# evandieren/AbstractBayesOpt.jl

Hardware: NVIDIA B200
Metric: candidate posterior+EI evals/sec at n=8192,d=20 (higher is better)
Workload: dtype f64

## Files before the change

abstractbayesopt.jl_b200/csrc/abo_api.cu:

```cuda
#include <algorithm>
#include <cmath>
#include <cstdarg>
#include <cstdio>
#include <cstring>
#include <cstdlib>
#include <limits>
#include <new>
#include <string>
#include <vector>

#include <cuda_runtime.h>

#include "../../include/abo.h"
#include "gemm_dmma.cuh"
#include "kernels.cuh"
#include "sweep_fused.cuh"
#include "gemm_tma.cuh"
#include "sample.cuh"
#include "abo_internal.h"

using namespace abo;

static thread_local std::string g_err;

int abo_fail(int code, const char* fmt, ...) {
    char buf[512];
    va_list ap;
    va_start(ap, fmt);
    vsnprintf(buf, sizeof buf, fmt, ap);
    va_end(ap);
    g_err = buf;
    return code;
}

extern "C" const char* abo_last_error(void) { return g_err.c_str(); }
extern "C" int32_t abo_version(void) { return 100; }

static int configure_kernels() {
    CU(cudaFuncSetAttribute(gemm_dmma_kernel, cudaFuncAttributeMaxDynamicSharedMemorySize, GEMM_SMEM_BYTES));
    CU(cudaFuncSetAttribute(gemm_small_kernel<32, 8>, cudaFuncAttributeMaxDynamicSharedMemorySize, GemmS<32, 8>::SMEM_BYTES));
    CU(cudaFuncSetAttribute(gemm_small_kernel<64, 8>, cudaFuncAttributeMaxDynamicSharedMemorySize, GemmS<64, 8>::SMEM_BYTES));
    CU(cudaFuncSetAttribute(gemm_k128_kernel<16, 128>, cudaFuncAttributeMaxDynamicSharedMemorySize, GemmK128<16, 128>::SMEM_BYTES));
    CU(cudaFuncSetAttribute(gemm_k128_kernel<32, 32>, cudaFuncAttributeMaxDynamicSharedMemorySize, GemmK128<32, 32>::SMEM_BYTES));
    CU(cudaFuncSetAttribute(fill_distance_kernel, cudaFuncAttributeMaxDynamicSharedMemorySize, 256 * 96 * 8));
    CU(cudaFuncSetAttribute(potf2_ws_kernel, cudaFuncAttributeMaxDynamicSharedMemorySize, PW_SMEM_BYTES));
    CU(cudaFuncSetAttribute(syrk_tma_kernel, cudaFuncAttributeMaxDynamicSharedMemorySize, SY_SMEM_BYTES));
    CU(cudaFuncSetAttribute(gemm_tma_kernel<EPI_STORE>, cudaFuncAttributeMaxDynamicSharedMemorySize, tg_smem_bytes<EPI_STORE>()));
    CU(cudaFuncSetAttribute(gemm_tma_kernel<EPI_COLSUMSQ>, cudaFuncAttributeMaxDynamicSharedMemorySize, tg_smem_bytes<EPI_COLSUMSQ>()));
#define ABO_FS_CFG(DT) CU(cudaFuncSetAttribute(sweep_fused_kernel<DT>, cudaFuncAttributeMaxDynamicSharedMemorySize, fused_smem_bytes<DT>()))
    ABO_FS_CFG(4); ABO_FS_CFG(8); ABO_FS_CFG(12); ABO_FS_CFG(16); ABO_FS_CFG(20); ABO_FS_CFG(24); ABO_FS_CFG(32);
#undef ABO_FS_CFG
    return ABO_OK;
}

static int ctx_init_resources(abo_ctx* c) {
    int prio_lo = 0, prio_hi = 0;
    CU(cudaDeviceGetStreamPriorityRange(&prio_lo, &prio_hi));
    CU(cudaStreamCreateWithPriority(&c->stream, cudaStreamNonBlocking, prio_hi));
    CU(cudaStreamCreateWithPriority(&c->stream2, cudaStreamNonBlocking, prio_lo));
    CU(cudaStreamCreateWithPriority(&c->stream3, cudaStreamNonBlocking, prio_hi));
    CU(cudaStreamCreateWithPriority(&c->stream4, cudaStreamNonBlocking, prio_lo));
    CU(cudaEventCreateWithFlags(&c->ev_inv, cudaEventDisableTiming));
    for (int q = 0; q < 3; ++q) CU(cudaEventCreateWithFlags(&c->ev_p[q], cudaEventDisableTiming));
    CU(cudaEventCreateWithFlags(&c->ev_a, cudaEventDisableTiming));
    CU(cudaEventCreateWithFlags(&c->ev_b, cudaEventDisableTiming));
    for (int q = 0; q < 2; ++q) {
        CU(cudaEventCreateWithFlags(&c->ev_h2d[q], cudaEventDisableTiming));
        CU(cudaEventCreateWithFlags(&c->ev_pc[q], cudaEventDisableTiming));
    }
    return configure_kernels();
}

extern "C" int32_t abo_ctx_create(int32_t device, abo_ctx** out) {
    if (!out) return abo_fail(ABO_ERR_INVALID, "abo_ctx_create: out is NULL");
    int ndev = 0;
    cudaError_t e = cudaGetDeviceCount(&ndev);
    if (e != cudaSuccess || ndev == 0)
        return abo_fail(ABO_ERR_CUDA, "no CUDA device available (%s); libabo_cuda has no CPU fallback",
                        e == cudaSuccess ? "device count 0" : cudaGetErrorString(e));
    if (device < 0 || device >= ndev) return abo_fail(ABO_ERR_INVALID, "device %d out of range [0,%d)", device, ndev);
    CU(cudaSetDevice(device));
    cudaDeviceProp prop;
    CU(cudaGetDeviceProperties(&prop, device));
    if (prop.major < 10)
        return abo_fail(ABO_ERR_CUDA, "device %d is sm_%d%d; libabo_cuda is built for sm_100a only", device, prop.major,
                        prop.minor);
    abo_ctx* c = new (std::nothrow) abo_ctx();
    if (!c) return abo_fail(ABO_ERR_ALLOC, "host allocation failed");
    c->device = device;
    c->sms = prop.multiProcessorCount;
    int rc = ctx_init_resources(c);
    if (rc) { abo_ctx_destroy(c); return rc; }
    *out = c;
    return ABO_OK;
}

static void gp_free_device(abo_gp* g);
void ctx_sync_all(abo_ctx* c) {
    for (cudaStream_t s_ : {c->stream, c->stream2, c->stream3, c->stream4}) if (s_) cudaStreamSynchronize(s_);
}

extern "C" int32_t abo_ctx_destroy(abo_ctx* c) {
    if (!c) return ABO_OK;
    const std::string keep = g_err;
    cudaSetDevice(c->device);
    ctx_sync_all(c);
    for (abo_gp* g : c->live) { gp_free_device(g); g->ctx = nullptr; }
    c->live.clear();
    for (auto& b : c->ws) if (b.ptr) cudaFree(b.ptr);
    gp_pool_clear(c);
    for (auto e : c->prof_events) cudaEventDestroy(e);
    if (c->pinned) cudaFreeHost(c->pinned);
    abo_nccl_teardown(c);
    auto ev_free = [](cudaEvent_t e) { if (e) cudaEventDestroy(e); };
    ev_free(c->ev_a); ev_free(c->ev_b);
    for (int q = 0; q < 2; ++q) { ev_free(c->ev_h2d[q]); ev_free(c->ev_pc[q]); }
    for (cudaStream_t s_ : {c->stream, c->stream2, c->stream3, c->stream4}) if (s_) cudaStreamDestroy(s_);
    ev_free(c->ev_inv);
    for (int q = 0; q < 3; ++q) ev_free(c->ev_p[q]);
    cudaGetLastError();
    delete c;
    g_err = keep;
    return ABO_OK;
}

extern "C" int32_t abo_ctx_trim(abo_ctx* c) {
    if (!c) return abo_fail(ABO_ERR_INVALID, "null ctx");
    CU(cudaSetDevice(c->device));
    ctx_sync_all(c);
    gp_pool_clear(c);
    for (auto& b : c->ws) if (b.ptr) { cudaFree(b.ptr); b.ptr = nullptr; b.bytes = 0; }
    if (c->pinned) { cudaFreeHost(c->pinned); c->pinned = nullptr; c->pinned_bytes = 0; }
    return ABO_OK;
}

extern "C" int32_t abo_ctx_device(const abo_ctx* c, int32_t* device) {
    if (!c || !device) return abo_fail(ABO_ERR_INVALID, "null argument");
    *device = c->device;
    return ABO_OK;
}
extern "C" int32_t abo_ctx_stream(const abo_ctx* c, void** stream) {
    if (!c || !stream) return abo_fail(ABO_ERR_INVALID, "null argument");
    *stream = (void*)c->stream;
    return ABO_OK;
}
extern "C" int32_t abo_ctx_launch_count(const abo_ctx* c, int64_t* count) {
    if (!c || !count) return abo_fail(ABO_ERR_INVALID, "null argument");
    *count = c->launches;
    return ABO_OK;
}

int prof_mark(abo_ctx* c) {
    if (!c->profile) return ABO_OK;
    if (c->prof_used == c->prof_events.size()) {
        cudaEvent_t e;
        CU(cudaEventCreate(&e));
        c->prof_events.push_back(e);
    }
    CU(cudaEventRecord(c->prof_events[c->prof_used++], c->stream));
    return ABO_OK;
}
int prof_collect(abo_ctx* c) {
    if (!c->profile) return ABO_OK;
    for (size_t i = 0; i + 1 < c->prof_used; i += 2) {
        float ms = 0;
        CU(cudaEventElapsedTime(&ms, c->prof_events[i], c->prof_events[i + 1]));
        int cls = (int)((i / 2) % 3);
        c->prof_ms[cls] += ms;
        c->prof_n[cls] += 1;
    }
    c->prof_used = 0;
    return ABO_OK;
}
extern "C" int32_t abo_ctx_profile(abo_ctx* c, int32_t enable) {
    if (!c) return abo_fail(ABO_ERR_INVALID, "null ctx");
    CU(cudaSetDevice(c->device));
    CU(cudaStreamSynchronize(c->stream));
    c->profile = enable != 0;
    c->prof_used = 0;
    for (int i = 0; i < 3; ++i) { c->prof_ms[i] = 0; c->prof_n[i] = 0; }
    return ABO_OK;
}
extern "C" int32_t abo_ctx_profile_read(abo_ctx* c, double ms[3], int64_t launches[3]) {
    if (!c || !ms || !launches) return abo_fail(ABO_ERR_INVALID, "null argument");
    CU(cudaSetDevice(c->device));
    CU(cudaStreamSynchronize(c->stream));
    int rc = prof_collect(c);
    if (rc) return rc;
    for (int i = 0; i < 3; ++i) { ms[i] = c->prof_ms[i]; launches[i] = c->prof_n[i]; }
    return ABO_OK;
}

typedef CUresult (*EncodeTiledFn)(CUtensorMap*, CUtensorMapDataType, cuuint32_t, void*, const cuuint64_t*,
                                  const cuuint64_t*, const cuuint32_t*, const cuuint32_t*, CUtensorMapInterleave,
                                  CUtensorMapSwizzle, CUtensorMapL2promotion, CUtensorMapFloatOOBfill);
static EncodeTiledFn get_encode_fn() {
    static EncodeTiledFn fn = nullptr;
    if (!fn) {
        void* ptr = nullptr;
        cudaDriverEntryPointQueryResult q;
        if (cudaGetDriverEntryPoint("cuTensorMapEncodeTiled", &ptr, cudaEnableDefault, &q) == cudaSuccess &&
            q == cudaDriverEntryPointSuccess)
            fn = (EncodeTiledFn)ptr;
    }
    return fn;
}
int make_tmap_k4(CUtensorMap* map, const double* base, int64_t K, int64_t rows, int64_t ld) {
    EncodeTiledFn fn = get_encode_fn();
    if (!fn) return abo_fail(ABO_ERR_CUDA, "cuTensorMapEncodeTiled is not available from this driver");
    cuuint64_t dims[2] = {(cuuint64_t)K, (cuuint64_t)rows};
    cuuint64_t strides[1] = {(cuuint64_t)ld * sizeof(double)};
    cuuint32_t box[2] = {4, 128};
    cuuint32_t estr[2] = {1, 1};
    CUresult r = fn(map, CU_TENSOR_MAP_DATA_TYPE_FLOAT64, 2, (void*)base, dims, strides, box, estr,
                    CU_TENSOR_MAP_INTERLEAVE_NONE, CU_TENSOR_MAP_SWIZZLE_NONE, CU_TENSOR_MAP_L2_PROMOTION_L2_256B,
                    CU_TENSOR_MAP_FLOAT_OOB_FILL_NONE);
    if (r != CUDA_SUCCESS) return abo_fail(ABO_ERR_CUDA, "cuTensorMapEncodeTiled failed with CUresult %d", (int)r);
    return ABO_OK;
}

extern "C" int32_t abo_debug_potf2_clocks(abo_ctx* c, int64_t out[16]) {
    if (!c || !out) return abo_fail(ABO_ERR_INVALID, "null argument");
    CU(cudaSetDevice(c->device));
    CU(cudaStreamSynchronize(c->stream));
    long long h[16];
    CU(cudaMemcpyFromSymbol(h, g_potf2_clk, sizeof h));
    for (int i = 0; i < 16; ++i) out[i] = h[i];
    return ABO_OK;
}

int ws_get(abo_ctx* c, int slot, size_t bytes, void** out) {
    auto& b = c->ws[slot];
    if (b.bytes < bytes) {
        if (b.ptr) { ctx_sync_all(c); CU(cudaFree(b.ptr)); b.ptr = nullptr; b.bytes = 0; }
        cudaError_t e = cudaMalloc(&b.ptr, bytes);
        if (e != cudaSuccess) { cudaGetLastError(); return abo_fail(ABO_ERR_ALLOC, "cudaMalloc(%zu) failed: %s", bytes, cudaGetErrorString(e)); }
        b.bytes = bytes;
    }
    *out = b.ptr;
    return ABO_OK;
}

void ws_release(abo_ctx* c, int slot) {
    auto& b = c->ws[slot];
    if (b.ptr) { ctx_sync_all(c); cudaFree(b.ptr); b.ptr = nullptr; b.bytes = 0; }
}

int pinned_get(abo_ctx* c, size_t bytes, void** out) {
    if (c->pinned_bytes < bytes) {
        if (c->pinned) { ctx_sync_all(c); cudaFreeHost(c->pinned); c->pinned = nullptr; c->pinned_bytes = 0; }
        cudaError_t e = cudaMallocHost(&c->pinned, bytes);
        if (e != cudaSuccess) { cudaGetLastError(); return abo_fail(ABO_ERR_ALLOC, "cudaMallocHost(%zu) failed", bytes); }
        c->pinned_bytes = bytes;
    }
    *out = c->pinned;
    return ABO_OK;
}

int make_tmap_k4(CUtensorMap* map, const double* base, int64_t K, int64_t rows, int64_t ld);
template <int EPI = EPI_STORE>
static int launch_gemm_tma(abo_ctx* c, const CUtensorMap& tmA, const CUtensorMap& tmB, TmaGemmParams p, cudaStream_t st, int max_ctas = 0);
int potrf_blocked(abo_ctx* c, double* A, int64_t Npad, int64_t ld, double* Dinv, int* info, int batch) {
    const int T = (int)(Npad / NB);
    const int64_t strideA = Npad * ld, strideD = (int64_t)T * NB * NB;
    cudaStream_t st = c->stream;
    CUtensorMap tmA, tmD;
    int rc;
    if ((rc = make_tmap_k4(&tmA, A, Npad, (int64_t)batch * Npad, ld)) || (rc = make_tmap_k4(&tmD, Dinv, NB, (int64_t)batch * T * NB, NB)))
        return rc;
    constexpr int OB = 2;
    for (int jb = 0; jb < T; ++jb) {
        double* Ajj = A + (int64_t)jb * NB * (ld + 1);
        double* Dj = Dinv + (int64_t)jb * NB * NB;
        potf2_ws_kernel<<<batch, 512, PW_SMEM_BYTES, st>>>(Ajj, ld, strideA, Dj, strideD, info, jb * NB);
        KL(c);
        const int rem = (int)(Npad - (int64_t)(jb + 1) * NB);
        if (rem <= 0) break;
        const int ob0 = jb / OB * OB, obend = std::min(ob0 + OB, T);
        TmaGemmParams g{};
        g.Mt = rem / NB; g.Nt = 1; g.batch = batch; g.K = NB; g.flags = 0; g.alpha = 1.0; g.beta = 0.0;
        g.a_row0 = (jb + 1) * NB; g.a_rstep = (int)Npad; g.a_col0 = jb * NB; g.a_cstep = 0;
        g.b_row0 = jb * NB; g.b_rstep = T * NB; g.b_col0 = 0; g.b_cstep = 0;
        g.C = A; g.ldc = ld; g.c_off0 = (int64_t)(jb + 1) * NB * ld + (int64_t)jb * NB; g.c_zstep = strideA;
        if ((rc = launch_gemm_tma(c, tmA, tmD, g, st))) return rc;
        const int nin = obend - jb - 1;
        if (nin > 0) {
            TmaGemmParams q{};
            q.Mt = rem / NB; q.Nt = nin; q.batch = batch; q.K = NB; q.flags = LOWER_ONLY; q.alpha = -1.0; q.beta = 1.0;
            q.a_row0 = (jb + 1) * NB; q.a_rstep = (int)Npad; q.a_col0 = jb * NB; q.a_cstep = 0;
            q.b_row0 = q.a_row0; q.b_rstep = q.a_rstep; q.b_col0 = q.a_col0; q.b_cstep = 0;
            q.C = A; q.ldc = ld; q.c_off0 = (int64_t)(jb + 1) * NB * (ld + 1); q.c_zstep = strideA;
            if ((rc = launch_gemm_tma(c, tmA, tmA, q, st))) return rc;
        }
        if (jb == obend - 1 && obend < T) {
            TmaGemmParams q{};
            q.Mt = T - obend; q.Nt = T - obend; q.batch = batch; q.K = (obend - ob0) * NB; q.flags = LOWER_ONLY; q.alpha = -1.0; q.beta = 1.0;
            q.a_row0 = obend * NB; q.a_rstep = (int)Npad; q.a_col0 = ob0 * NB; q.a_cstep = 0;
            q.b_row0 = q.a_row0; q.b_rstep = q.a_rstep; q.b_col0 = q.a_col0; q.b_cstep = 0;
            q.C = A; q.ldc = ld; q.c_off0 = (int64_t)obend * NB * (ld + 1); q.c_zstep = strideA;
            if ((rc = launch_gemm_tma(c, tmA, tmA, q, st))) return rc;
        }
    }
    return ABO_OK;
}

template <typename... KArgs, typename... Args>
static cudaError_t launch_pdl(void (*kernel)(KArgs...), dim3 grid, dim3 block, size_t smem, cudaStream_t st, bool pdl,
                              Args... args) {
    cudaLaunchConfig_t cfg = {};
    cfg.gridDim = grid; cfg.blockDim = block; cfg.dynamicSmemBytes = smem; cfg.stream = st;
    cudaLaunchAttribute attr[1];
    attr[0].id = cudaLaunchAttributeProgrammaticStreamSerialization;
    attr[0].val.programmaticStreamSerializationAllowed = 1;
    cfg.attrs = attr; cfg.numAttrs = pdl ? 1 : 0;
    return cudaLaunchKernelEx(&cfg, kernel, KArgs(args)...);
}

constexpr int LA_OB = 3;
constexpr int LA_PDL_TILES = 40;
constexpr int LA_SMALL_NEXT = 60;
constexpr int LA_BIG_REM = 4096;
int potrf_lookahead(abo_ctx* c, double* A, int64_t Npad, int64_t ld, double* Dinv, int* info, int notify_tile, cudaStream_t notify_stream) {
    const int T = (int)(Npad / NB);
    cudaStream_t sp = c->stream, su = c->stream2;
    CUtensorMap tmL;
    int rc = make_tmap_k4(&tmL, A, Npad, Npad, ld);
    if (rc) return rc;
    CU(cudaEventRecord(c->ev_a, sp));
    CU(cudaStreamWaitEvent(su, c->ev_a, 0));
    bool rest_pending = false;
    bool s3_pending = false;
    bool boundary_split = false;
    cudaStream_t s3 = c->stream3;
    int step = 0;
    for (int Jb = 0, je = 0; Jb < T; Jb = je, ++step) {
        je = std::min(Jb + std::min(step + 1, LA_OB), T);
        const bool pdl = (T - Jb) <= LA_PDL_TILES;
        for (int jp = Jb; jp < je; ++jp) {
            double* Ajj = A + (int64_t)jp * NB * (ld + 1);
            double* Dj = Dinv + (int64_t)jp * NB * NB;
            CU(launch_pdl(potf2_ws_kernel, dim3(1), dim3(512), PW_SMEM_BYTES, sp, pdl, Ajj, ld, (int64_t)0, Dj, (int64_t)0, info, jp * NB));
            KL(c);
            if (s3_pending) { CU(cudaStreamWaitEvent(sp, c->ev_p[2], 0)); s3_pending = false; }
            const int rem = (T - jp - 1) * NB;
            if (rem <= 0) break;
            double* P = Ajj + (int64_t)NB * ld;
            const int ncol = (je - jp - 1) * NB;
            auto gemm_panel = [&](const GemmParams& q, cudaStream_t s_, bool pdl_) -> int {
                if (q.M <= 0 || q.N <= 0) return ABO_OK;
                if (q.M >= LA_BIG_REM) CU(launch_pdl(gemm_small_kernel<64, 8>, dim3(q.N / BN, q.M / 64, 1), dim3(256), GemmS<64, 8>::SMEM_BYTES, s_, pdl_, q));
                else CU(launch_pdl(gemm_small_kernel<32, 8>, dim3(q.N / BN, q.M / 32, 1), dim3(256), GemmS<32, 8>::SMEM_BYTES, s_, pdl_, q));
                KL(c);
                return ABO_OK;
            };
            GemmParams g{};
            g.A = P; g.lda = ld; g.B = Dj; g.ldb = NB; g.C = P; g.ldc = ld;
            g.M = rem; g.N = NB; g.K = NB; g.alpha = 1.0; g.beta = 0.0; g.flags = 0;
            GemmParams s{};
            s.A = P; s.lda = ld; s.B = P; s.ldb = ld;
            s.C = Ajj + (int64_t)NB * (ld + 1); s.ldc = ld;
            s.M = rem; s.N = ncol; s.K = NB; s.alpha = -1.0; s.beta = 1.0; s.flags = LOWER_ONLY;
            int rc2;
            if (ncol <= 0 && rem > NB) {
                GemmParams g1 = g; g1.M = NB;
                CU(launch_pdl(gemm_k128_kernel<16, 128>, dim3(1, 8, 1), dim3(128), GemmK128<16, 128>::SMEM_BYTES, sp, pdl, g1)); KL(c);
                CU(cudaEventRecord(c->ev_p[1], sp));
                CU(cudaStreamWaitEvent(s3, c->ev_p[1], 0));
                GemmParams g2 = g; g2.A = P + (int64_t)NB * ld; g2.C = P + (int64_t)NB * ld; g2.M = rem - NB;
                if ((rc2 = gemm_panel(g2, s3, false))) return rc2;
                CU(cudaEventRecord(c->ev_p[2], s3));
                s3_pending = true;
                boundary_split = true;
            } else if (ncol <= 0 || rem <= NB) {
                if ((rc2 = gemm_panel(g, sp, pdl))) return rc2;
                if ((rc2 = gemm_panel(s, sp, pdl))) return rc2;
            } else {
                GemmParams g1 = g; g1.M = NB;
                GemmParams s1 = s; s1.M = NB; s1.N = NB; s1.flags = 0;
                CU(launch_pdl(gemm_k128_kernel<16, 128>, dim3(1, 8, 1), dim3(128), GemmK128<16, 128>::SMEM_BYTES, sp, pdl, g1)); KL(c);
                CU(launch_pdl(gemm_k128_kernel<32, 32>, dim3(4, 4, 1), dim3(128), GemmK128<32, 32>::SMEM_BYTES, sp, pdl, s1)); KL(c);
                CU(cudaEventRecord(c->ev_p[1], sp));
                CU(cudaStreamWaitEvent(s3, c->ev_p[1], 0));
                GemmParams g2 = g; g2.A = P + (int64_t)NB * ld; g2.C = P + (int64_t)NB * ld; g2.M = rem - NB;
                if ((rc2 = gemm_panel(g2, s3, false))) return rc2;
                GemmParams s2 = s;
                s2.A = P + (int64_t)NB * ld; s2.C = s.C + (int64_t)NB * ld; s2.M = rem - NB; s2.lower_shift = NB;
                if ((rc2 = gemm_panel(s2, s3, false))) return rc2;
                CU(cudaEventRecord(c->ev_p[2], s3));
                s3_pending = true;
            }
        }
        if (s3_pending && !boundary_split) { CU(cudaStreamWaitEvent(sp, c->ev_p[2], 0)); s3_pending = false; }
        if (je >= T) break;
        SyrkParams u;
        u.C = A; u.ld = ld; u.kcol0 = Jb * NB; u.nk = (je - Jb) * (NB / 16); u.skip_first = 0;
        const int jn = std::min(je + std::min(step + 2, LA_OB), T);
        CU(cudaEventRecord(c->ev_a, sp));
        if (notify_stream && notify_tile > 0 && je >= notify_tile) {
            CU(cudaStreamWaitEvent(notify_stream, c->ev_a, 0));
            if (boundary_split) CU(cudaStreamWaitEvent(notify_stream, c->ev_p[2], 0));
            notify_tile = 0;
        }
        if (jn < T) {
            CU(cudaStreamWaitEvent(su, c->ev_a, 0));
            if (boundary_split) CU(cudaStreamWaitEvent(su, c->ev_p[2], 0));
            u.row_t0 = jn; u.col_t0 = jn;
            syrk_tma_kernel<<<dim3(T - jn, T - jn), SW_THREADS, SY_SMEM_BYTES, su>>>(tmL, u);
            KL(c);
        }
        if (rest_pending) CU(cudaStreamWaitEvent(sp, c->ev_b, 0));
        cudaStream_t sn = sp;
        bool pdl_next = pdl && !rest_pending;
        if (boundary_split) {
            GemmParams dn{};
            dn.A = A + (int64_t)je * NB * ld + (int64_t)Jb * NB; dn.lda = ld;
            dn.B = dn.A; dn.ldb = ld;
            dn.C = A + (int64_t)je * NB * (ld + 1); dn.ldc = ld;
            dn.M = NB; dn.N = NB; dn.K = (je - Jb) * NB; dn.alpha = -1.0; dn.beta = 1.0; dn.flags = 0;
            CU(launch_pdl(gemm_k128_kernel<32, 32>, dim3(4, 4, 1), dim3(128), GemmK128<32, 32>::SMEM_BYTES, sp, pdl_next, dn)); KL(c);
            if (rest_pending) CU(cudaStreamWaitEvent(s3, c->ev_b, 0));
            sn = s3; pdl_next = false; u.skip_first = 1;
        }
        if ((T - je) * (jn - je) <= LA_SMALL_NEXT) {
            GemmParams nx{};
            nx.A = A + (int64_t)je * NB * ld + (int64_t)Jb * NB; nx.lda = ld;
            nx.B = nx.A; nx.ldb = ld;
            nx.C = A + (int64_t)je * NB * (ld + 1); nx.ldc = ld;
            nx.M = (T - je) * NB; nx.N = (jn - je) * NB; nx.K = (je - Jb) * NB;
            nx.alpha = -1.0; nx.beta = 1.0; nx.flags = LOWER_ONLY | (boundary_split ? SKIP_FIRST : 0);
            CU(launch_pdl(gemm_small_kernel<32, 8>, dim3(nx.N / BN, nx.M / 32, 1), dim3(256), GemmS<32, 8>::SMEM_BYTES, sn,
                          pdl_next, nx));
        } else {
            u.row_t0 = je; u.col_t0 = je;
            CU(launch_pdl(syrk_tma_kernel, dim3(jn - je, T - je), dim3(SW_THREADS), SY_SMEM_BYTES, sn, pdl_next, tmL, u));
        }
        KL(c);
        if (boundary_split) {
            CU(cudaEventRecord(c->ev_p[2], s3));
            s3_pending = true;
            boundary_split = false;
        }
        if (jn < T) { CU(cudaEventRecord(c->ev_b, su)); rest_pending = true; }
    }
    if (rest_pending) CU(cudaStreamWaitEvent(sp, c->ev_b, 0));
    if (notify_stream && notify_tile > 0) {
        CU(cudaEventRecord(c->ev_a, sp));
        CU(cudaStreamWaitEvent(notify_stream, c->ev_a, 0));
    }
    return ABO_OK;
}

__global__ void place_diag_both_kernel(const double* __restrict__ Dinv, double* __restrict__ Linv, double* __restrict__ U, int64_t ld,
                                       int64_t strideD, int64_t strideL) {
    const int t = blockIdx.x;
    const double* src = Dinv + (int64_t)blockIdx.y * strideD + (int64_t)t * NB * NB;
    double* dst = Linv + (int64_t)blockIdx.y * strideL + (int64_t)t * NB * (ld + 1);
    double* dsu = U + (int64_t)blockIdx.y * strideL + (int64_t)t * NB * (ld + 1);
    for (int e = threadIdx.x; e < NB * NB; e += blockDim.x) {
        const int r = e >> 7, cc = e & 127;
        dst[(int64_t)r * ld + cc] = src[e];
        dsu[(int64_t)r * ld + cc] = src[cc * NB + r];
    }
}
template <int EPI>
static int launch_gemm_tma(abo_ctx* c, const CUtensorMap& tmA, const CUtensorMap& tmB, TmaGemmParams p, cudaStream_t st, int max_ctas) {
    if (p.Mt <= 0 || p.Nt <= 0 || p.batch <= 0) return ABO_OK;
    if ((p.flags & LOWER_ONLY) && p.Nt > p.Mt) return abo_fail(ABO_ERR_INVALID, "gemm_tma: LOWER_ONLY needs Nt <= Mt");
    const int64_t per = (p.flags & LOWER_ONLY) ? (int64_t)p.Nt * (p.Nt + 1) / 2 + (int64_t)(p.Mt - p.Nt) * p.Nt : (int64_t)p.Mt * p.Nt;
    const int64_t total = per * p.batch;
    if (total > 0x7fffffff) return abo_fail(ABO_ERR_INVALID, "too many tiles in one launch");
    p.total = (int)total;
    gemm_tma_kernel<EPI><<<(int)std::min<int64_t>(total, max_ctas > 0 ? max_ctas : c->sms), SW_THREADS, tg_smem_bytes<EPI>(), st>>>(tmA, tmB, p);
    KL(c);
    return ABO_OK;
}
struct TrtriPair { int o, b, rr, zb, rstep, cstep; int64_t zoff; };
static int trtri_pair_w(abo_ctx* c, const CUtensorMap& tmL, const CUtensorMap& tmU, double* Wt, int64_t ld, const TrtriPair& q,
                        cudaStream_t st, int max_ctas) {
    TmaGemmParams g{};
    g.batch = q.zb; g.alpha = 1.0; g.beta = 0.0;
    g.Mt = q.rr; g.Nt = q.b; g.K = q.b * NB; g.flags = KLO_N;
    g.a_row0 = (q.o + q.b) * NB; g.a_col0 = q.o * NB; g.a_rstep = q.rstep; g.a_cstep = q.cstep;
    g.b_row0 = q.o * NB; g.b_col0 = q.o * NB; g.b_rstep = q.rstep; g.b_cstep = q.cstep;
    g.C = nullptr; g.CT = Wt; g.ldct = ld; g.ct_off0 = (int64_t)q.o * NB * ld + (int64_t)(q.o + q.b) * NB; g.ct_zstep = q.zoff;
    return launch_gemm_tma(c, tmL, tmU, g, st, max_ctas);
}
static int trtri_pair_x(abo_ctx* c, const CUtensorMap& tmX, const CUtensorMap& tmW, double* Linv, double* U, int64_t ld,
                        const TrtriPair& q, cudaStream_t st, int max_ctas) {
    TmaGemmParams h{};
    h.batch = q.zb; h.alpha = -1.0; h.beta = 0.0;
    h.Mt = q.rr; h.Nt = q.b; h.K = q.rr * NB; h.flags = KHI_M;
    h.a_row0 = (q.o + q.b) * NB; h.a_col0 = (q.o + q.b) * NB; h.a_rstep = q.rstep; h.a_cstep = q.cstep;
    h.b_row0 = q.o * NB; h.b_col0 = (q.o + q.b) * NB; h.b_rstep = q.rstep; h.b_cstep = q.cstep;
    h.C = Linv; h.ldc = ld; h.c_off0 = (int64_t)(q.o + q.b) * NB * ld + (int64_t)q.o * NB; h.c_zstep = q.zoff;
    h.CT = U; h.ldct = ld; h.ct_off0 = (int64_t)q.o * NB * ld + (int64_t)(q.o + q.b) * NB; h.ct_zstep = q.zoff;
    return launch_gemm_tma(c, tmX, tmW, h, st, max_ctas);
}
static int trtri_tma_on(abo_ctx* c, const double* L, double* Linv, double* U, double* Wt, int64_t Npad, int64_t ld, int64_t strideM,
                        const double* Dinv, int64_t strideD, int batch, cudaStream_t st, int max_ctas) {
    const int T = (int)(Npad / NB);
    const int64_t rows = (batch == 1) ? Npad : (int64_t)batch * Npad;
    if (batch > 1 && strideM != Npad * ld) return abo_fail(ABO_ERR_INVALID, "trtri_tma: batched matrices must be contiguous");
    place_diag_both_kernel<<<dim3(T, batch), 256, 0, st>>>(Dinv, Linv, U, ld, strideD, strideM);
    KL(c);
    if (T == 1) return ABO_OK;
    CUtensorMap tmL, tmX, tmU, tmW;
    int rc;
    if ((rc = make_tmap_k4(&tmL, L, Npad, rows, ld)) || (rc = make_tmap_k4(&tmX, Linv, Npad, rows, ld)) ||
        (rc = make_tmap_k4(&tmU, U, Npad, rows, ld)) || (rc = make_tmap_k4(&tmW, Wt, Npad, rows, ld)))
        return rc;
    for (int b = 1; b < T; b <<= 1) {
        const int npairs = (T - b + 2 * b - 1) / (2 * b), nfull = T / (2 * b);
        struct Grp { int q0, nq, rr; };
        std::vector<Grp> groups;
        if (nfull > 0) groups.push_back({0, nfull, b});
        if (npairs > nfull) groups.push_back({nfull, 1, T - 2 * b * nfull - b});
        for (const Grp& gq : groups) {
            const int launches = (batch == 1) ? 1 : gq.nq;
            for (int li = 0; li < launches; ++li) {
                TrtriPair q;
                q.o = 2 * b * (gq.q0 + li); q.b = b; q.rr = gq.rr;
                q.zb = (batch == 1) ? gq.nq : batch;
                q.rstep = (batch == 1) ? 2 * b * NB : (int)Npad; q.cstep = (batch == 1) ? 2 * b * NB : 0;
                q.zoff = (batch == 1) ? (int64_t)2 * b * NB * (ld + 1) : strideM;
                if ((rc = trtri_pair_w(c, tmL, tmU, Wt, ld, q, st, max_ctas)) || (rc = trtri_pair_x(c, tmX, tmW, Linv, U, ld, q, st, max_ctas)))
                    return rc;
            }
        }
    }
    return ABO_OK;
}
int trtri_tma(abo_ctx* c, const double* L, double* Linv, double* U, double* Wt, int64_t Npad, int64_t ld, int64_t strideM,
              const double* Dinv, int64_t strideD, int batch) {
    return trtri_tma_on(c, L, Linv, U, Wt, Npad, ld, strideM, Dinv, strideD, batch, c->stream, 0);
}

int solve_alpha(abo_ctx* c, const double* Linv, int64_t ld, int64_t N, const double* delta, double* beta,
                double* alpha, int64_t strideM, int64_t strideV, int batch) {
    cudaStream_t st = c->stream;
    {
        int64_t threads = N * 32;
        dim3 grid((unsigned)((threads + 255) / 256), batch);
        trmv_lower_kernel<<<grid, 256, 0, st>>>(Linv, ld, N, delta, beta, strideM, strideV);
        KL(c);
    }
    const int nchunks = (int)((N + TRMVT_ROWS - 1) / TRMVT_ROWS);
    double* part;
    int rc = ws_get(c, WS_VEC_PART, sizeof(double) * (size_t)nchunks * N * batch, (void**)&part);
    if (rc) return rc;
    {
        dim3 grid((unsigned)((N + 127) / 128), nchunks, batch);
        trmvT_lower_partial_kernel<<<grid, 128, 0, st>>>(Linv, ld, N, beta, part, strideM, strideV, (int64_t)nchunks * N);
        KL(c);
        dim3 g2((unsigned)((N + 127) / 128), batch);
        reduce_rows_kernel<<<g2, 128, 0, st>>>(part, nchunks, N, alpha, (int64_t)nchunks * N, strideV);
        KL(c);
    }
    return ABO_OK;
}

constexpr size_t GP_POOL_MAX_SETS = 3;
constexpr size_t GP_POOL_MAX_BYTES = (size_t)24 << 30;
static size_t gp_set_bytes(int64_t cap_pad) { return 2 * sizeof(double) * (size_t)cap_pad * cap_pad; }

static void gp_free_device(abo_gp* g) {
    cudaSetDevice(g->ctx->device);
    double** ptrs[] = {&g->dXsT, &g->dL, &g->dLinv, &g->dAlpha, &g->dBeta, &g->dDelta, &g->dMeanC};
    if (g->share && --*g->share == 0) {
        delete g->share;
        abo_ctx* c = g->ctx;
        size_t pooled = 0;
        for (auto& e : c->gp_pool) pooled += gp_set_bytes(e.cap_pad);
        if (g->dL && c->gp_pool.size() < GP_POOL_MAX_SETS && pooled + gp_set_bytes(g->cap_pad) <= GP_POOL_MAX_BYTES) {
            abo_ctx::GpBufSet e{g->cap_pad, g->ldx, g->d, g->p, {}};
            for (int q = 0; q < 7; ++q) e.ptr[q] = *ptrs[q];
            c->gp_pool.push_back(e);
        } else {
            for (auto pp : ptrs) if (*pp) cudaFree(*pp);
        }
    }
    for (auto pp : ptrs) *pp = nullptr;
    g->share = nullptr;
    g->fitted = false;
    g->cap_pad = 0;
}

void gp_pool_clear(abo_ctx* c) {
    for (auto& e : c->gp_pool) for (double* q : e.ptr) if (q) cudaFree(q);
    c->gp_pool.clear();
}

int gp_alloc(abo_gp* g, int64_t Npad, int64_t ldx) {
    gp_free_device(g);
    abo_ctx* c = g->ctx;
    double** ptrs[] = {&g->dXsT, &g->dL, &g->dLinv, &g->dAlpha, &g->dBeta, &g->dDelta, &g->dMeanC};
    g->share = new (std::nothrow) int(1);
    if (!g->share) return abo_fail(ABO_ERR_ALLOC, "host allocation failed");
    for (size_t q = 0; q < c->gp_pool.size(); ++q) {
        auto& e = c->gp_pool[q];
        if (e.cap_pad == Npad && e.ldx == ldx && e.d == g->d && e.p == g->p) {
            for (int r = 0; r < 7; ++r) *ptrs[r] = e.ptr[r];
            c->gp_pool.erase(c->gp_pool.begin() + q);
            g->cap_pad = Npad; g->ld = Npad; g->ldx = ldx;
            return ABO_OK;
        }
    }
    size_t mat = sizeof(double) * (size_t)Npad * Npad;
    cudaError_t e = cudaSuccess;
    for (int attempt = 0; attempt < 2; ++attempt) {
        if ((e = cudaMalloc(&g->dL, mat)) == cudaSuccess && (e = cudaMalloc(&g->dLinv, mat)) == cudaSuccess &&
            (e = cudaMalloc(&g->dXsT, sizeof(double) * (size_t)ldx * g->d)) == cudaSuccess &&
            (e = cudaMalloc(&g->dAlpha, sizeof(double) * Npad)) == cudaSuccess &&
            (e = cudaMalloc(&g->dBeta, sizeof(double) * Npad)) == cudaSuccess &&
            (e = cudaMalloc(&g->dDelta, sizeof(double) * Npad)) == cudaSuccess &&
            (e = cudaMalloc(&g->dMeanC, sizeof(double) * g->p)) == cudaSuccess)
            break;
        cudaGetLastError();
        for (auto pp : ptrs) { if (*pp) cudaFree(*pp); *pp = nullptr; }
        if (attempt == 0 && !c->gp_pool.empty()) { gp_pool_clear(c); continue; }
        delete g->share; g->share = nullptr;
        return abo_fail(ABO_ERR_ALLOC, "device allocation for a %lld x %lld posterior failed: %s", (long long)Npad,
                        (long long)Npad, cudaGetErrorString(e));
    }
    g->cap_pad = Npad;
    g->ld = Npad;
    g->ldx = ldx;
    return ABO_OK;
}

__global__ void copy_lower_tiles_kernel(const double* __restrict__ a0, const double* __restrict__ a1, double* __restrict__ b0,
                                        double* __restrict__ b1, int64_t ld) {
    if (blockIdx.x > blockIdx.y) return;
    const double* src = blockIdx.z ? a1 : a0;
    double* dst = blockIdx.z ? b1 : b0;
    const int64_t base = (int64_t)blockIdx.y * NB * ld + (int64_t)blockIdx.x * NB;
    for (int e = threadIdx.x; e < NB * NB / 2; e += blockDim.x) {
        const int r = e / (NB / 2), c2 = e % (NB / 2);
        reinterpret_cast<double2*>(dst + base + (int64_t)r * ld)[c2] = reinterpret_cast<const double2*>(src + base + (int64_t)r * ld)[c2];
    }
}

int gp_unshare(abo_gp* g) {
    if (!gp_shared(g)) return ABO_OK;
    abo_ctx* c = g->ctx;
    cudaStream_t st = c->stream;
    abo_gp old = *g;
    g->dXsT = g->dL = g->dLinv = g->dAlpha = g->dBeta = g->dDelta = g->dMeanC = nullptr;
    g->share = nullptr;
    const bool fitted = old.fitted;
    int rc = gp_alloc(g, old.cap_pad, old.ldx);
    if (rc) { *g = old; return rc; }
    const int T = (int)(old.cap_pad / NB);
    copy_lower_tiles_kernel<<<dim3(T, T, 2), 256, 0, st>>>(old.dL, old.dLinv, g->dL, g->dLinv, old.ld);
    KL(c);
    CU(cudaMemcpyAsync(g->dXsT, old.dXsT, sizeof(double) * old.ldx * old.d, cudaMemcpyDeviceToDevice, st));
    CU(cudaMemcpyAsync(g->dAlpha, old.dAlpha, sizeof(double) * old.cap_pad, cudaMemcpyDeviceToDevice, st));
    CU(cudaMemcpyAsync(g->dBeta, old.dBeta, sizeof(double) * old.cap_pad, cudaMemcpyDeviceToDevice, st));
    CU(cudaMemcpyAsync(g->dDelta, old.dDelta, sizeof(double) * old.cap_pad, cudaMemcpyDeviceToDevice, st));
    CU(cudaMemcpyAsync(g->dMeanC, old.dMeanC, sizeof(double) * old.p, cudaMemcpyDeviceToDevice, st));
    CU(cudaStreamSynchronize(st));
    --*old.share;
    g->fitted = fitted;
    return ABO_OK;
}

extern "C" int32_t abo_gp_create(abo_ctx* ctx, int32_t kernel_id, int32_t d, int32_t p, abo_gp** out) {
    if (!ctx || !out) return abo_fail(ABO_ERR_INVALID, "null argument");
    if (kernel_id < 0 || kernel_id > 6) return abo_fail(ABO_ERR_INVALID, "unknown kernel id %d", kernel_id);
    if (d < 1) return abo_fail(ABO_ERR_INVALID, "d must be >= 1");
    if (p != 1 && p != d + 1) return abo_fail(ABO_ERR_INVALID, "p must be 1 (StandardGP) or d+1 (GradientGP)");
    if (p > 1 && (kernel_id == ABO_KERNEL_MATERN52 || kernel_id == ABO_KERNEL_MATERN72))
        return abo_fail(ABO_ERR_INVALID,
                        "KernelFunctions Matern kernels are not differentiable at 0 (NaN, test/test_kernels.jl:87); "
                        "use the Approx/AD variants for GradientGP");
    abo_gp* g = new (std::nothrow) abo_gp();
    if (!g) return abo_fail(ABO_ERR_ALLOC, "host allocation failed");
    g->ctx = ctx; g->kind = kernel_id; g->d = d; g->p = p;
    g->s = 1.0; g->scale = 1.0; g->noise = 0.0;
    g->sv.assign(d, 1.0); g->ard = false;
    g->mean_c.assign(p, 0.0);
    ctx->live.insert(g);
    *out = g;
    return ABO_OK;
}

extern "C" int32_t abo_gp_destroy(abo_gp* g) {
    if (!g) return ABO_OK;
    if (g->ctx) { g->ctx->live.erase(g); gp_free_device(g); }
    delete g;
    return ABO_OK;
}

extern "C" int32_t abo_gp_set_params(abo_gp* g, double inv_ls, double scale, double noise, const double* mean_c) {
    if (!g) return abo_fail(ABO_ERR_INVALID, "null gp");
    if (!(inv_ls > 0) || !(scale > 0) || !(noise >= 0) || !std::isfinite(inv_ls) || !std::isfinite(scale))
        return abo_fail(ABO_ERR_INVALID, "hyper-parameters must be positive and finite (noise >= 0)");
    g->s = inv_ls; g->scale = scale; g->noise = noise;
    g->sv.assign(g->d, inv_ls); g->ard = false;
    for (int a = 0; a < g->p; ++a) g->mean_c[a] = mean_c ? mean_c[a] : 0.0;
    g->fitted = false;
    return ABO_OK;
}

extern "C" int32_t abo_gp_set_params_ard(abo_gp* g, const double* inv_ls, double scale, double noise, const double* mean_c) {
    if (!g || !inv_ls) return abo_fail(ABO_ERR_INVALID, "null argument");
    if (g->d > ARD_MAXD) return abo_fail(ABO_ERR_INVALID, "ARD length scales are supported for d <= %d", ARD_MAXD);
    for (int k = 0; k < g->d; ++k)
        if (!(inv_ls[k] > 0) || !std::isfinite(inv_ls[k])) return abo_fail(ABO_ERR_INVALID, "inverse length scales must be positive and finite");
    if (!(scale > 0) || !(noise >= 0) || !std::isfinite(scale)) return abo_fail(ABO_ERR_INVALID, "hyper-parameters must be positive and finite (noise >= 0)");
    g->sv.assign(inv_ls, inv_ls + g->d);
    g->s = inv_ls[0]; g->scale = scale; g->noise = noise; g->ard = true;
    for (int a = 0; a < g->p; ++a) g->mean_c[a] = mean_c ? mean_c[a] : 0.0;
    g->fitted = false;
    return ABO_OK;
}

static KSpec gp_spec(const abo_gp* g) {
    KSpec k;
    k.kind = g->kind; k.d = g->d; k.p = g->p; k.s = g->s; k.scale = g->scale; k.noise = g->noise;
    for (int q = 0; q < ARD_MAXD; ++q) k.sv[q] = (q < g->d && q < (int)g->sv.size()) ? g->sv[q] : g->s;
    return k;
}

static int gp_fit_run(abo_gp* g, const double* X, const double* y, int64_t n, int64_t* info_out);
constexpr int FIT_OVERLAP_MIN_TILES = 32;
constexpr int FIT_OVERLAP_CTAS = 112;
extern "C" int32_t abo_gp_fit(abo_gp* g, const double* X, const double* y, int64_t n, int64_t* info_out) {
    const int rc = gp_fit_run(g, X, y, n, info_out);
    if (rc && g && g->ctx) {
        const std::string keep = g_err;
        ctx_sync_all(g->ctx);
        cudaGetLastError();
        g_err = keep;
    }
    return rc;
}
static int gp_fit_run(abo_gp* g, const double* X, const double* y, int64_t n, int64_t* info_out) {
    if (!g || !X || !y) return abo_fail(ABO_ERR_INVALID, "null argument");
    if (n < 1) return abo_fail(ABO_ERR_DIM, "need at least one observation");
    if (!g->ctx) return abo_fail(ABO_ERR_INVALID, "the context of this handle has been destroyed");
    abo_ctx* c = g->ctx;
    CU(cudaSetDevice(c->device));
    cudaStream_t st = c->stream;
    const int64_t N = n * g->p;
    const int64_t Npad = (N + NB - 1) / NB * NB;
    const int64_t ldx = (n + NB - 1) / NB * NB + NB;
    g->fitted = false;
    if (Npad != g->cap_pad || ldx > g->ldx || gp_shared(g)) { int rc = gp_alloc(g, Npad, ldx); if (rc) return rc; }
    g->n = n; g->N = N; g->Npad = Npad;

    double *dXraw, *dYraw;
    int rc;
    if ((rc = ws_get(c, WS_STAGE_X, sizeof(double) * (size_t)n * g->d, (void**)&dXraw))) return rc;
    if ((rc = ws_get(c, WS_STAGE_Y, sizeof(double) * (size_t)N, (void**)&dYraw))) return rc;
    CU(cudaMemcpyAsync(dXraw, X, sizeof(double) * n * g->d, cudaMemcpyHostToDevice, st));
    CU(cudaMemcpyAsync(dYraw, y, sizeof(double) * N, cudaMemcpyHostToDevice, st));
    CU(cudaMemcpyAsync(g->dMeanC, g->mean_c.data(), sizeof(double) * g->p, cudaMemcpyHostToDevice, st));
    {
        int64_t tot = g->ldx * g->d;
        scale_transpose_kernel<<<(unsigned)((tot + 255) / 256), 256, 0, st>>>(dXraw, g->dXsT, n, g->d, g->ldx, gp_spec(g));
        KL(c);
        fill_kernel<<<(unsigned)((Npad + 255) / 256), 256, 0, st>>>(g->dDelta, Npad, 0.0);
        KL(c);
        delta_kernel<<<(unsigned)((N + 255) / 256), 256, 0, st>>>(dYraw, g->dMeanC, n, g->p, g->dDelta);
        KL(c);
    }
    const int T = (int)(Npad / NB);
    KmatBatch bt{nullptr, nullptr, 0, 0, 0};
    launch_kmat(gp_spec(g), g->dXsT, g->ldx, N, g->dL, g->ld, bt, T, 1, st);
    KL(c);

    double* Dinv; int* dinfo; double* W;
    if ((rc = ws_get(c, WS_DINV, sizeof(double) * (size_t)T * NB * NB, (void**)&Dinv))) return rc;
    if ((rc = ws_get(c, WS_INFO, sizeof(int) * 16, (void**)&dinfo))) return rc;
    if ((rc = ws_get(c, WS_TRTRI, sizeof(double) * (size_t)Npad * Npad, (void**)&W))) return rc;
    CU(cudaMemsetAsync(dinfo, 0, sizeof(int) * 16, st));
    double* U;
    if ((rc = ws_get(c, WS_TRTRI_U, sizeof(double) * (size_t)Npad * Npad, (void**)&U))) return rc;
    int b_top = 1;
    while (2 * b_top < T) b_top *= 2;
    const TrtriPair top{0, b_top, T - b_top, 1, 0, 0, 0};
    const bool overlap = T >= FIT_OVERLAP_MIN_TILES;
    if ((rc = potrf_lookahead(c, g->dL, Npad, g->ld, Dinv, dinfo, overlap ? b_top : 0, overlap ? c->stream4 : nullptr))) return rc;
    if (overlap) {
        cudaStream_t s4 = c->stream4;
        const int64_t nl = (int64_t)b_top * NB;
        if ((rc = trtri_tma_on(c, g->dL, g->dLinv, U, W, nl, g->ld, 0, Dinv, 0, 1, s4, FIT_OVERLAP_CTAS))) return rc;
        CUtensorMap tmL, tmU;
        if ((rc = make_tmap_k4(&tmL, g->dL, Npad, Npad, g->ld)) || (rc = make_tmap_k4(&tmU, U, Npad, Npad, g->ld))) return rc;
        if ((rc = trtri_pair_w(c, tmL, tmU, W, g->ld, top, s4, FIT_OVERLAP_CTAS))) return rc;
        CU(cudaEventRecord(c->ev_inv, s4));
    }
    int hinfo = 0;
    CU(cudaMemcpyAsync(&hinfo, dinfo, sizeof(int), cudaMemcpyDeviceToHost, st));
    CU(cudaStreamSynchronize(st));
    if (info_out) *info_out = hinfo;
    if (hinfo != 0)
        return abo_fail(ABO_ERR_NOT_POSDEF, "matrix is not positive definite; Cholesky factorization failed at pivot %d", hinfo);
    if (overlap) {
        const int64_t off = (int64_t)b_top * NB * (g->ld + 1);
        if ((rc = trtri_tma_on(c, g->dL + off, g->dLinv + off, U + off, W + off, Npad - (int64_t)b_top * NB, g->ld, 0,
                               Dinv + (int64_t)b_top * NB * NB, 0, 1, st, 0))) return rc;
        CU(cudaStreamWaitEvent(st, c->ev_inv, 0));
        CUtensorMap tmX, tmW;
        if ((rc = make_tmap_k4(&tmX, g->dLinv, Npad, Npad, g->ld)) || (rc = make_tmap_k4(&tmW, W, Npad, Npad, g->ld))) return rc;
        if ((rc = trtri_pair_x(c, tmX, tmW, g->dLinv, U, g->ld, top, st, 0))) return rc;
    } else if ((rc = trtri_tma(c, g->dL, g->dLinv, U, W, Npad, g->ld, 0, Dinv, 0, 1))) return rc;
    if ((rc = solve_alpha(c, g->dLinv, g->ld, Npad, g->dDelta, g->dBeta, g->dAlpha, 0, 0, 1))) return rc;
    CU(cudaStreamSynchronize(st));
    g->fitted = true;
    return ABO_OK;
}

extern "C" int32_t abo_gp_clone(const abo_gp* g, abo_gp** out) {
    if (!g || !out) return abo_fail(ABO_ERR_INVALID, "null argument");
    abo_gp* n = new (std::nothrow) abo_gp(*g);
    if (!n) return abo_fail(ABO_ERR_ALLOC, "host allocation failed");
    if (n->share) ++*n->share;
    if (n->ctx) n->ctx->live.insert(n);
    *out = n;
    return ABO_OK;
}

extern "C" int32_t abo_gp_n(const abo_gp* g, int64_t* n) {
    if (!g || !n) return abo_fail(ABO_ERR_INVALID, "null argument");
    *n = g->fitted ? g->n : 0;
    return ABO_OK;
}

extern "C" int32_t abo_gp_alpha(const abo_gp* g, double* alpha) {
    if (!g || !alpha) return abo_fail(ABO_ERR_INVALID, "null argument");
    if (!g->fitted) return abo_fail(ABO_ERR_NOT_FITTED, "surrogate has no posterior");
    abo_ctx* c = g->ctx;
    CU(cudaSetDevice(c->device));
    double* tmp;
    int rc = ws_get(c, WS_STAGE_Y, sizeof(double) * (size_t)g->N, (void**)&tmp);
    if (rc) return rc;
    to_out_major_kernel<<<(unsigned)((g->N + 255) / 256), 256, 0, c->stream>>>(g->dAlpha, g->n, g->p, tmp);
    KL(c);
    CU(cudaMemcpyAsync(alpha, tmp, sizeof(double) * g->N, cudaMemcpyDeviceToHost, c->stream));
    CU(cudaStreamSynchronize(c->stream));
    return ABO_OK;
}

extern "C" int32_t abo_gp_factor(const abo_gp* g, int32_t which, double* out) {
    if (!g || !out) return abo_fail(ABO_ERR_INVALID, "null argument");
    if (!g->fitted) return abo_fail(ABO_ERR_NOT_FITTED, "surrogate has no posterior");
    CU(cudaSetDevice(g->ctx->device));
    const double* src = which == 0 ? g->dL : g->dLinv;
    CU(cudaMemcpy2DAsync(out, sizeof(double) * g->N, src, sizeof(double) * g->ld, sizeof(double) * g->N, g->N,
                         cudaMemcpyDeviceToHost, g->ctx->stream));
    CU(cudaStreamSynchronize(g->ctx->stream));
    for (int64_t i = 0; i < g->N; ++i)
        for (int64_t j = i + 1; j < g->N; ++j) out[i * g->N + j] = 0.0;
    return ABO_OK;
}

template <int DT>
static void launch_ks(abo_ctx* c, const abo_gp* g, const double* dXc, int64_t c_begin, int64_t m_total, int bo,
                      double* Ks, double* pmean, int64_t mc_eff, int64_t mc, int npb, cudaStream_t stream) {
    if (g->p == 1)
        ks_build_kernel<DT, false><<<dim3(npb, (unsigned)(mc_eff / KS_CB)), 128, 0, stream>>>(
            gp_spec(g), g->dXsT, g->ldx, g->n, g->N, g->Npad, g->dAlpha, dXc, c_begin, m_total, bo, Ks, pmean, mc);
    else
        ks_build_kernel<DT, true><<<dim3(npb, (unsigned)(mc_eff / KS_CB)), 128, 0, stream>>>(
            gp_spec(g), g->dXsT, g->ldx, g->n, g->N, g->Npad, g->dAlpha, dXc, c_begin, m_total, bo, Ks, pmean, mc);
}

static int launch_ks_d(abo_ctx* c, const abo_gp* g, const double* dXc, int64_t c0, int64_t m, int bo, double* Ks, double* pmean,
                       int64_t mc_eff, int64_t mc, int npb, cudaStream_t st) {
    const int d = g->d;
    if (d <= 4) launch_ks<4>(c, g, dXc, c0, m, bo, Ks, pmean, mc_eff, mc, npb, st);
    else if (d <= 8) launch_ks<8>(c, g, dXc, c0, m, bo, Ks, pmean, mc_eff, mc, npb, st);
    else if (d <= 12) launch_ks<12>(c, g, dXc, c0, m, bo, Ks, pmean, mc_eff, mc, npb, st);
    else if (d <= 16) launch_ks<16>(c, g, dXc, c0, m, bo, Ks, pmean, mc_eff, mc, npb, st);
    else if (d <= 20) launch_ks<20>(c, g, dXc, c0, m, bo, Ks, pmean, mc_eff, mc, npb, st);
    else if (d <= 24) launch_ks<24>(c, g, dXc, c0, m, bo, Ks, pmean, mc_eff, mc, npb, st);
    else if (d <= 32) launch_ks<32>(c, g, dXc, c0, m, bo, Ks, pmean, mc_eff, mc, npb, st);
    else
        ks_build_generic_kernel<<<dim3(npb, (unsigned)(mc_eff / KS_CB)), 128, 0, st>>>(
            gp_spec(g), g->dXsT, g->ldx, g->n, g->N, g->Npad, g->dAlpha, dXc, c0, m, bo, Ks, pmean, mc);
    KL(c);
    return ABO_OK;
}

static double phi_prime0(int kind) {
    if (kind == K_SE) return -0.5;
    if (kind == K_M52 || kind == K_AM52 || kind == K_ADM52) return -5.0 / 6.0;
    return -7.0 / 10.0;
}

static bool fused_applies(const abo_gp* g, int bo) {
    return g->p == 1 && bo == 0 && g->d <= 32 && g->Npad <= FS_MAX_NPAD;
}
static int sweep_fused_device(abo_gp* g, const double* dXc, int64_t m, const AcqSpec& a, double* d_mean, double* d_var,
                              double* d_score) {
    abo_ctx* c = g->ctx;
    cudaStream_t st = c->stream;
    FusedParams fp;
    fp.spec = gp_spec(g); fp.acq = a;
    fp.XsT = g->dXsT; fp.ldx = g->ldx; fp.n = g->n;
    fp.T = (int)((g->n + NB - 1) / NB);
    fp.Kld = (int)((g->n + 15) / 16 * 16);
    fp.Xc = dXc; fp.m = m; fp.beta = g->dBeta;
    fp.mean_out = d_mean; fp.var_out = d_var; fp.score_out = d_score;
    fp.ntiles = (int)((m + NB - 1) / NB);
    const int grid = std::min(c->sms, fp.ntiles);
    int rc;
    if ((rc = ws_get(c, WS_KS, sizeof(double) * (size_t)c->sms * 2 * NB * fp.Kld, (void**)&fp.scratch))) return rc;
    CUtensorMap tmA, tmB;
    if ((rc = make_tmap_k4(&tmA, g->dLinv, g->Npad, g->Npad, g->ld))) return rc;
    if ((rc = make_tmap_k4(&tmB, fp.scratch, fp.Kld, (int64_t)c->sms * 2 * NB, fp.Kld))) return rc;
    if ((rc = prof_mark(c)) || (rc = prof_mark(c))) return rc;
    if ((rc = prof_mark(c))) return rc;
#define ABO_FS_RUN(DT) sweep_fused_kernel<DT><<<grid, FS_THREADS, fused_smem_bytes<DT>(), st>>>(tmA, tmB, fp)
    const int d = g->d;
    if (d <= 4) ABO_FS_RUN(4); else if (d <= 8) ABO_FS_RUN(8); else if (d <= 12) ABO_FS_RUN(12); else if (d <= 16) ABO_FS_RUN(16);
    else if (d <= 20) ABO_FS_RUN(20); else if (d <= 24) ABO_FS_RUN(24); else ABO_FS_RUN(32);
#undef ABO_FS_RUN
    KL(c);
    if ((rc = prof_mark(c))) return rc;
    if ((rc = prof_mark(c)) || (rc = prof_mark(c))) return rc;
    if (c->profile && c->prof_used >= 6 * 512) {
        CU(cudaStreamSynchronize(st));
        if ((rc = prof_collect(c))) return rc;
    }
    return ABO_OK;
}

int sweep_device(abo_gp* g, const double* dXc, int64_t m, int bo, int acq, const double* params, double* d_mean,
                 double* d_var, double* d_score) {
    abo_ctx* c = g->ctx;
    cudaStream_t st = c->stream;
    {
        AcqSpec a0;
        a0.acq = acq;
        a0.p0 = params ? params[0] : 0.0;
        a0.p1 = (params && acq != ACQ_UCB && acq >= 0) ? params[1] : 0.0;
        a0.mean_c = g->mean_c[bo];
        a0.kss = g->scale;
        if (fused_applies(g, bo)) return sweep_fused_device(g, dXc, m, a0, d_mean, d_var, d_score);
    }
    const int64_t Npad = g->Npad;
    const int T = (int)(Npad / NB);
    int64_t mc = (int64_t)NB * ((2048 + T - 1) / T);
    mc = std::min<int64_t>(mc, ((int64_t)(512ll << 20) / (Npad * 8)) / NB * NB);
    mc = std::max<int64_t>(NB, std::min<int64_t>(mc, 65536));
    mc = std::min<int64_t>(mc, (m + NB - 1) / NB * NB);
    const int64_t vpts = (Npad + g->p - 1) / g->p;
    const int npb = (int)((vpts + 127) / 128);
    double *Ks, *pmean, *sumsq;
    int rc;
    if ((rc = ws_get(c, WS_KS, sizeof(double) * (size_t)mc * Npad, (void**)&Ks))) return rc;
    if ((rc = ws_get(c, WS_PMEAN, sizeof(double) * (size_t)npb * mc, (void**)&pmean))) return rc;
    if ((rc = ws_get(c, WS_SUMSQ, sizeof(double) * (size_t)T * mc, (void**)&sumsq))) return rc;
    CUtensorMap tmA, tmB;
    if ((rc = make_tmap_k4(&tmA, g->dLinv, Npad, Npad, g->ld))) return rc;
    if ((rc = make_tmap_k4(&tmB, Ks, Npad, mc, Npad))) return rc;
    AcqSpec a;
    a.acq = acq;
    a.p0 = params ? params[0] : 0.0;
    a.p1 = (params && acq != ACQ_UCB && acq >= 0) ? params[1] : 0.0;
    a.mean_c = g->mean_c[bo];
    const double sb_ = (bo > 0 && bo - 1 < (int)g->sv.size() && g->d <= ARD_MAXD) ? g->sv[bo - 1] : g->s;
    a.kss = (bo == 0) ? g->scale : -2.0 * sb_ * sb_ * g->scale * phi_prime0(g->kind);
    for (int64_t c0 = 0; c0 < m; c0 += mc) {
        const int64_t mvalid = std::min(mc, m - c0);
        const int64_t mc_eff = (mvalid + NB - 1) / NB * NB;
        if ((rc = prof_mark(c))) return rc;
        if ((rc = launch_ks_d(c, g, dXc, c0, m, bo, Ks, pmean, mc_eff, mc, npb, st))) return rc;
        if ((rc = prof_mark(c))) return rc;
        if ((rc = prof_mark(c))) return rc;
        TmaGemmParams sp{};
        sp.batch = 1; sp.Mt = T; sp.Nt = (int)(mc_eff / NB); sp.K = (int)Npad; sp.flags = KHI_M;
        sp.C = sumsq; sp.ldc = mc;
        if ((rc = launch_gemm_tma<EPI_COLSUMSQ>(c, tmA, tmB, sp, st))) return rc;
        if ((rc = prof_mark(c))) return rc;
        if ((rc = prof_mark(c))) return rc;
        acq_epilogue_kernel<<<(unsigned)((mvalid + 255) / 256), 256, 0, st>>>(
            a, pmean, npb, sumsq, T, mc, mvalid, d_mean ? d_mean + c0 : nullptr, d_var ? d_var + c0 : nullptr,
            d_score ? d_score + c0 : nullptr);
        KL(c);
        if ((rc = prof_mark(c))) return rc;
        if (c->profile && c->prof_used >= 6 * 512) {
            CU(cudaStreamSynchronize(st));
            if ((rc = prof_collect(c))) return rc;
        }
    }
    CU(cudaGetLastError());
    return ABO_OK;
}

constexpr int64_t HOST_PIECE = 262144;
static int sweep_host_pieces(abo_gp* g, const double* Xc, int64_t m, int acq_id, const double* params, double* h_mean,
                             double* h_var, double* h_scores, int64_t k, int64_t* top_idx, double* top_val);

extern "C" int32_t abo_gp_posterior(abo_gp* g, const double* Xc, int64_t m, int32_t outputs, double* mean, double* var) {
    if (!g || !Xc) return abo_fail(ABO_ERR_INVALID, "null argument");
    if (!g->fitted) return abo_fail(ABO_ERR_NOT_FITTED, "surrogate has no posterior (call update first)");
    if (outputs != 1 && outputs != g->p) return abo_fail(ABO_ERR_INVALID, "outputs must be 1 or p");
    if (m <= 0) return ABO_OK;
    abo_ctx* c = g->ctx;
    CU(cudaSetDevice(c->device));
    if (outputs == 1 && m > HOST_PIECE && !c->profile)
        return sweep_host_pieces(g, Xc, m, -1, nullptr, mean, var, nullptr, 0, nullptr, nullptr);
    cudaStream_t st = c->stream;
    double *dXc, *dm, *dv;
    int rc;
    if ((rc = ws_get(c, WS_CAND, sizeof(double) * (size_t)m * g->d, (void**)&dXc))) return rc;
    if ((rc = ws_get(c, WS_OUT_A, sizeof(double) * (size_t)m * outputs, (void**)&dm))) return rc;
    if ((rc = ws_get(c, WS_OUT_B, sizeof(double) * (size_t)m * outputs, (void**)&dv))) return rc;
    CU(cudaMemcpyAsync(dXc, Xc, sizeof(double) * m * g->d, cudaMemcpyHostToDevice, st));
    for (int bo = 0; bo < outputs; ++bo)
        if ((rc = sweep_device(g, dXc, m, bo, -1, nullptr, dm + (int64_t)bo * m, dv + (int64_t)bo * m, nullptr))) return rc;
    if (mean) CU(cudaMemcpyAsync(mean, dm, sizeof(double) * m * outputs, cudaMemcpyDeviceToHost, st));
    if (var) CU(cudaMemcpyAsync(var, dv, sizeof(double) * m * outputs, cudaMemcpyDeviceToHost, st));
    CU(cudaStreamSynchronize(st));
    return ABO_OK;
}

static int linv_times_ks(abo_ctx* c, const abo_gp* g, const double* Ks, int64_t ncol, double* W, cudaStream_t st, double* Wt = nullptr) {
    CUtensorMap tmX, tmK;
    int rc;
    if ((rc = make_tmap_k4(&tmX, g->dLinv, g->Npad, g->Npad, g->ld)) || (rc = make_tmap_k4(&tmK, Ks, g->Npad, ncol, g->Npad))) return rc;
    TmaGemmParams w{};
    w.batch = 1; w.alpha = 1.0; w.beta = 0.0; w.Mt = (int)(g->Npad / NB); w.Nt = (int)(ncol / NB); w.K = (int)g->Npad; w.flags = KHI_M;
    w.C = W; w.ldc = ncol;
    w.CT = Wt; w.ldct = g->Npad;
    return launch_gemm_tma(c, tmX, tmK, w, st);
}

extern "C" int32_t abo_acq_eval_grad(abo_gp* g, int32_t acq_id, const double* params, const double* Xc, int64_t m,
                                     double* scores, double* grad, double* mean, double* var) {
    if (!g || !Xc || !params || !scores || !grad) return abo_fail(ABO_ERR_INVALID, "null argument");
    if (!g->fitted) return abo_fail(ABO_ERR_NOT_FITTED, "surrogate has no posterior (call update first)");
    if (acq_id < 0 || acq_id > 2) return abo_fail(ABO_ERR_INVALID, "unknown acquisition id %d", acq_id);
    if (g->d > AG_MAXD) return abo_fail(ABO_ERR_INVALID, "abo_acq_eval_grad supports d <= %d", AG_MAXD);
    if (m <= 0) return ABO_OK;
    abo_ctx* c = g->ctx;
    CU(cudaSetDevice(c->device));
    cudaStream_t st = c->stream;
    const int64_t Npad = g->Npad;
    const int d = g->d;
    const int64_t mc = 2048;
    const int64_t vpts = (Npad + g->p - 1) / g->p;
    const int npb = (int)((vpts + 127) / 128);
    const int npbg = (int)((g->n + 127) / 128);
    double *dXc, *Ks, *pmean, *W, *Z, *part, *out;
    int rc;
    if ((rc = ws_get(c, WS_CAND, sizeof(double) * (size_t)m * d, (void**)&dXc))) return rc;
    if ((rc = ws_get(c, WS_KS, sizeof(double) * (size_t)mc * Npad, (void**)&Ks))) return rc;
    if ((rc = ws_get(c, WS_PMEAN, sizeof(double) * (size_t)npb * mc, (void**)&pmean))) return rc;
    if ((rc = ws_get(c, WS_GRAD_W, sizeof(double) * (size_t)mc * Npad, (void**)&W))) return rc;
    if ((rc = ws_get(c, WS_GRAD_Z, sizeof(double) * (size_t)mc * Npad, (void**)&Z))) return rc;
    if ((rc = ws_get(c, WS_GRAD_PART, sizeof(double) * (size_t)npbg * mc * 2 * AG_MAXD, (void**)&part))) return rc;
    if ((rc = ws_get(c, WS_GRAD_OUT, sizeof(double) * (size_t)(mc + 3 * m + m * d), (void**)&out))) return rc;
    double *colsq = out, *dS = out + mc, *dM = dS + m, *dV = dM + m, *dG = dV + m;
    CU(cudaMemcpyAsync(dXc, Xc, sizeof(double) * m * d, cudaMemcpyHostToDevice, st));
    AcqSpec a;
    a.acq = acq_id;
    a.p0 = params[0];
    a.p1 = (acq_id != ACQ_UCB) ? params[1] : 0.0;
    a.mean_c = g->mean_c[0];
    a.kss = g->scale;
    for (int64_t c0 = 0; c0 < m; c0 += mc) {
        const int64_t mvalid = std::min(mc, m - c0);
        const int64_t mpad = (mvalid + NB - 1) / NB * NB;
        if ((rc = launch_ks_d(c, g, dXc, c0, m, 0, Ks, pmean, mpad, mc, npb, st))) return rc;
        KL(c);
        if ((rc = linv_times_ks(c, g, Ks, mpad, W, st))) return rc;
        colsumsq_kernel<<<(unsigned)((mpad + 127) / 128), 128, 0, st>>>(W, Npad, mpad, colsq);
        KL(c);
        GemmParams z{};
        z.A = g->dLinv; z.lda = g->ld; z.B = W; z.ldb = mpad; z.C = Z; z.ldc = mpad;
        z.M = (int)Npad; z.N = (int)mpad; z.K = (int)Npad; z.alpha = 1.0; z.beta = 0.0; z.flags = KLO_M;
        CU((launch_gemm(z, 1, st)));
        KL(c);
        acq_grad_partial_kernel<<<dim3(npbg, (unsigned)mpad), 128, 0, st>>>(gp_spec(g), g->dXsT, g->ldx, g->n, g->dAlpha, Z,
                                                                           mpad, dXc + c0 * d, mvalid, part);
        KL(c);
        acq_grad_finish_kernel<<<(unsigned)((mvalid + 127) / 128), 128, 0, st>>>(a, d, pmean, npb, colsq, part, npbg, mc, mpad,
                                                                                 mvalid, dS + c0, dG + c0 * d, dM + c0, dV + c0);
        KL(c);
    }
    CU(cudaMemcpyAsync(scores, dS, sizeof(double) * m, cudaMemcpyDeviceToHost, st));
    CU(cudaMemcpyAsync(grad, dG, sizeof(double) * m * d, cudaMemcpyDeviceToHost, st));
    if (mean) CU(cudaMemcpyAsync(mean, dM, sizeof(double) * m, cudaMemcpyDeviceToHost, st));
    if (var) CU(cudaMemcpyAsync(var, dV, sizeof(double) * m, cudaMemcpyDeviceToHost, st));
    CU(cudaStreamSynchronize(st));
    return ABO_OK;
}

extern "C" int32_t abo_gp_posterior_cov(abo_gp* g, const double* Xc, int64_t m, int32_t outputs, double* cov) {
    if (!g || !Xc || !cov) return abo_fail(ABO_ERR_INVALID, "null argument");
    if (!g->fitted) return abo_fail(ABO_ERR_NOT_FITTED, "surrogate has no posterior (call update first)");
    if (outputs != 1 && outputs != g->p) return abo_fail(ABO_ERR_INVALID, "outputs must be 1 or p");
    if (m <= 0) return ABO_OK;
    const int64_t mp = (m + KS_CB - 1) / KS_CB * KS_CB;
    const int64_t Mtot = mp * outputs, Mpad = (Mtot + NB - 1) / NB * NB;
    if (m * outputs > 8192) return abo_fail(ABO_ERR_INVALID, "posterior covariance is limited to m*outputs <= 8192");
    abo_ctx* c = g->ctx;
    CU(cudaSetDevice(c->device));
    cudaStream_t st = c->stream;
    const int64_t Npad = g->Npad;
    const int d = g->d;
    const int64_t vpts = (Npad + g->p - 1) / g->p;
    const int npb = (int)((vpts + 127) / 128);
    double *dXc, *Ks, *pmean, *W, *G, *dcov;
    int rc;
    if ((rc = ws_get(c, WS_CAND, sizeof(double) * (size_t)m * d, (void**)&dXc))) return rc;
    if ((rc = ws_get(c, WS_KS, sizeof(double) * (size_t)Mpad * Npad, (void**)&Ks))) return rc;
    if ((rc = ws_get(c, WS_PMEAN, sizeof(double) * (size_t)npb * Mpad, (void**)&pmean))) return rc;
    if ((rc = ws_get(c, WS_GRAD_W, sizeof(double) * (size_t)Mpad * Npad, (void**)&W))) return rc;
    if ((rc = ws_get(c, WS_GRAD_Z, sizeof(double) * (size_t)Mpad * Mpad, (void**)&G))) return rc;
    if ((rc = ws_get(c, WS_GRAD_OUT, sizeof(double) * (size_t)(m * outputs) * (m * outputs), (void**)&dcov))) return rc;
    CU(cudaMemcpyAsync(dXc, Xc, sizeof(double) * m * d, cudaMemcpyHostToDevice, st));
    CU(cudaMemsetAsync(Ks, 0, sizeof(double) * (size_t)Mpad * Npad, st));
    for (int bo = 0; bo < outputs; ++bo) {
        double* Kb = Ks + (size_t)bo * mp * Npad;
        double* pm = pmean + (size_t)bo * mp;
        if ((rc = launch_ks_d(c, g, dXc, 0, m, bo, Kb, pm, mp, Mpad, npb, st))) return rc;
    }
    if ((rc = linv_times_ks(c, g, Ks, Mpad, W, st))) return rc;
    GemmParams q{};
    q.A = W; q.lda = Mpad; q.B = W; q.ldb = Mpad; q.C = G; q.ldc = Mpad;
    q.M = (int)Mpad; q.N = (int)Mpad; q.K = (int)Npad; q.alpha = 1.0; q.beta = 0.0; q.flags = 0;
    CU((launch_gemm(q, 1, st)));
    KL(c);
    const int64_t Mo = m * outputs;
    cov_finish_kernel<<<(unsigned)((Mo * Mo + 255) / 256), 256, 0, st>>>(gp_spec(g), dXc, m, outputs, mp, G, Mpad, dcov, Mo, 0, 0.0);
    KL(c);
    CU(cudaMemcpyAsync(cov, dcov, sizeof(double) * Mo * Mo, cudaMemcpyDeviceToHost, st));
    CU(cudaStreamSynchronize(st));
    return ABO_OK;
}

constexpr int64_t SAMPLE_MAX_M = 16384, SAMPLE_MAX_S = 4096;
constexpr int SAMPLE_JITTER_STEPS = 7;
static int gp_posterior_sample_run(abo_gp* g, const double* Xc, int64_t m, int64_t S, uint64_t seed, double jitter,
                                   double* samples, int64_t* argmin_idx, double* argmin_val, double* jitter_used);
extern "C" int32_t abo_gp_posterior_sample(abo_gp* g, const double* Xc, int64_t m, int64_t S, uint64_t seed, double jitter,
                                           double* samples, int64_t* argmin_idx, double* argmin_val, double* jitter_used) {
    const int rc = gp_posterior_sample_run(g, Xc, m, S, seed, jitter, samples, argmin_idx, argmin_val, jitter_used);
    if (rc && g && g->ctx) {
        const std::string keep = g_err;
        ctx_sync_all(g->ctx);
        cudaGetLastError();
        g_err = keep;
    }
    return rc;
}
static int gp_posterior_sample_run(abo_gp* g, const double* Xc, int64_t m, int64_t S, uint64_t seed, double jitter,
                                   double* samples, int64_t* argmin_idx, double* argmin_val, double* jitter_used) {
    if (!g || !Xc) return abo_fail(ABO_ERR_INVALID, "null argument");
    if (!g->fitted) return abo_fail(ABO_ERR_NOT_FITTED, "surrogate has no posterior (call update first)");
    if (!(jitter > 0) || !std::isfinite(jitter)) return abo_fail(ABO_ERR_INVALID, "jitter must be positive and finite");
    if (m > SAMPLE_MAX_M || S > SAMPLE_MAX_S)
        return abo_fail(ABO_ERR_INVALID, "joint samples are limited to m <= %lld candidates and S <= %lld draws",
                        (long long)SAMPLE_MAX_M, (long long)SAMPLE_MAX_S);
    if (m <= 0 || S <= 0) return ABO_OK;
    abo_ctx* c = g->ctx;
    CU(cudaSetDevice(c->device));
    cudaStream_t st = c->stream;
    const int64_t Npad = g->Npad, Mpad = (m + NB - 1) / NB * NB, Spad = (S + NB - 1) / NB * NB;
    const int T = (int)(Mpad / NB);
    const int npb = (int)(((Npad + g->p - 1) / g->p + 127) / 128);
    double *dXc, *Ks, *pmean, *Wt, *G, *Sig, *Z, *F, *mu, *amin, *Dinv;
    int* dinfo;
    int rc;
    if ((rc = ws_get(c, WS_CAND, sizeof(double) * (size_t)m * g->d, (void**)&dXc)) ||
        (rc = ws_get(c, WS_KS, sizeof(double) * (size_t)Mpad * Npad, (void**)&Ks)) ||
        (rc = ws_get(c, WS_PMEAN, sizeof(double) * (size_t)npb * Mpad, (void**)&pmean)) ||
        (rc = ws_get(c, WS_GRAD_W, sizeof(double) * (size_t)Mpad * Npad, (void**)&Wt)) ||
        (rc = ws_get(c, WS_SAMPLE_G, sizeof(double) * (size_t)Mpad * Mpad, (void**)&G)) ||
        (rc = ws_get(c, WS_SAMPLE_SIGMA, sizeof(double) * (size_t)Mpad * Mpad, (void**)&Sig)) ||
        (rc = ws_get(c, WS_SAMPLE_Z, sizeof(double) * (size_t)Spad * Mpad, (void**)&Z)) ||
        (rc = ws_get(c, WS_SAMPLE_F, sizeof(double) * (size_t)Spad * Mpad, (void**)&F)) ||
        (rc = ws_get(c, WS_OUT_B, sizeof(double) * (size_t)Mpad, (void**)&mu)) ||
        (rc = ws_get(c, WS_OUT_A, sizeof(double) * (size_t)2 * S, (void**)&amin)) ||
        (rc = ws_get(c, WS_DINV, sizeof(double) * (size_t)T * NB * NB, (void**)&Dinv)) ||
        (rc = ws_get(c, WS_INFO, sizeof(int) * 16, (void**)&dinfo)))
        return rc;
    CU(cudaMemcpyAsync(dXc, Xc, sizeof(double) * m * g->d, cudaMemcpyHostToDevice, st));
    if ((rc = launch_ks_d(c, g, dXc, 0, m, 0, Ks, pmean, Mpad, Mpad, npb, st))) return rc;
    if ((rc = linv_times_ks(c, g, Ks, Mpad, nullptr, st, Wt))) return rc;
    {
        CUtensorMap tmW;
        if ((rc = make_tmap_k4(&tmW, Wt, Npad, Mpad, Npad))) return rc;
        TmaGemmParams q{};
        q.Mt = T; q.Nt = T; q.batch = 1; q.K = (int)Npad; q.flags = LOWER_ONLY; q.alpha = 1.0; q.beta = 0.0;
        q.C = G; q.ldc = Mpad;
        if ((rc = launch_gemm_tma(c, tmW, tmW, q, st))) return rc;
    }
    {
        AcqSpec a{};
        a.acq = -1; a.mean_c = g->mean_c[0]; a.kss = g->scale;
        acq_epilogue_kernel<<<(unsigned)((m + 255) / 256), 256, 0, st>>>(a, pmean, npb, nullptr, 0, Mpad, m, mu, nullptr, nullptr);
        KL(c);
    }
    philox_normal_kernel<<<(unsigned)((Spad * Mpad / 4 + 255) / 256), 256, 0, st>>>(seed, S, m, Spad, Mpad, Z);
    KL(c);
    double tau = 0.0;
    for (int k = 0;; ++k) {
        double p10 = 1.0;
        for (int e = 0; e < k; ++e) p10 *= 10.0;
        tau = jitter * g->scale * p10;
        cov_finish_kernel<<<(unsigned)((Mpad * Mpad + 255) / 256), 256, 0, st>>>(gp_spec(g), dXc, m, 1, Mpad, G, Mpad, Sig, Mpad,
                                                                                 Mpad, tau);
        KL(c);
        CU(cudaMemsetAsync(dinfo, 0, sizeof(int) * 16, st));
        if ((rc = potrf_lookahead(c, Sig, Mpad, Mpad, Dinv, dinfo))) return rc;
        int hinfo = 0;
        CU(cudaMemcpyAsync(&hinfo, dinfo, sizeof(int), cudaMemcpyDeviceToHost, st));
        CU(cudaStreamSynchronize(st));
        if (hinfo == 0) break;
        ctx_sync_all(c);
        if (k + 1 == SAMPLE_JITTER_STEPS)
            return abo_fail(ABO_ERR_NOT_POSDEF, "posterior covariance + %g I is not positive definite (pivot %d)", tau, hinfo);
    }
    zero_diag_upper_kernel<<<T, 256, 0, st>>>(Sig, Mpad);
    KL(c);
    {
        CUtensorMap tmL, tmZ;
        if ((rc = make_tmap_k4(&tmL, Sig, Mpad, Mpad, Mpad)) || (rc = make_tmap_k4(&tmZ, Z, Mpad, Spad, Mpad))) return rc;
        TmaGemmParams f{};
        f.Mt = T; f.Nt = (int)(Spad / NB); f.batch = 1; f.K = (int)Mpad; f.flags = KHI_M; f.alpha = 1.0; f.beta = 0.0;
        f.C = nullptr; f.CT = F; f.ldct = Mpad;
        if ((rc = launch_gemm_tma(c, tmL, tmZ, f, st))) return rc;
    }
    long long* aidx = reinterpret_cast<long long*>(amin);
    sample_finish_kernel<<<(unsigned)S, SF_THREADS, 0, st>>>(F, Mpad, mu, m, aidx, amin + S);
    KL(c);
    if (samples)
        CU(cudaMemcpy2DAsync(samples, sizeof(double) * m, F, sizeof(double) * Mpad, sizeof(double) * m, S, cudaMemcpyDeviceToHost, st));
    if (argmin_idx) CU(cudaMemcpyAsync(argmin_idx, aidx, sizeof(int64_t) * S, cudaMemcpyDeviceToHost, st));
    if (argmin_val) CU(cudaMemcpyAsync(argmin_val, amin + S, sizeof(double) * S, cudaMemcpyDeviceToHost, st));
    CU(cudaStreamSynchronize(st));
    if (jitter_used) *jitter_used = tau;
    return ABO_OK;
}


struct SelSlot { SelState* st; unsigned int* ties; unsigned long long* excl; long long* idx; double* val; };
static int sel_slot(abo_ctx* c, int slot, int64_t max_m, int64_t max_k, SelSlot* out) {
    const size_t nblk = (size_t)((max_m + SEL_CHUNK - 1) / SEL_CHUNK);
    const size_t a0 = (sizeof(SelState) + 255) / 256 * 256, a1 = (nblk * 4 + 255) / 256 * 256, a2 = (nblk * 8 + 255) / 256 * 256,
                 a3 = ((size_t)max_k * 8 + 255) / 256 * 256;
    const size_t per = a0 + a1 + a2 + 2 * a3;
    char* base;
    int rc = ws_get(c, WS_SELECT, 2 * per, (void**)&base);
    if (rc) return rc;
    base += (size_t)slot * per;
    out->st = (SelState*)base; out->ties = (unsigned int*)(base + a0); out->excl = (unsigned long long*)(base + a0 + a1);
    out->idx = (long long*)(base + a0 + a1 + a2); out->val = (double*)(base + a0 + a1 + a2 + a3);
    return ABO_OK;
}
static int device_topk_launch(abo_ctx* c, const SelSlot& q, const double* dS, int64_t m, int64_t K, cudaStream_t st) {
    const int nblk = (int)((m + SEL_CHUNK - 1) / SEL_CHUNK);
    const int hgrid = (int)std::min<int64_t>((m + 255) / 256, (int64_t)c->sms * 8);
    sel_init_kernel<<<1, 256, 0, st>>>(q.st, (long long)K);
    KL(c);
    for (int pass = 0; pass < 8; ++pass) {
        sel_hist_kernel<<<hgrid, 256, 0, st>>>(dS, m, pass, q.st);
        KL(c);
        sel_pick_kernel<<<1, 256, 0, st>>>(q.st);
        KL(c);
    }
    sel_tiecount_kernel<<<nblk, 256, 0, st>>>(dS, m, q.st, q.ties);
    KL(c);
    sel_tiescan_kernel<<<1, 32, 0, st>>>(q.ties, nblk, q.excl);
    KL(c);
    sel_gather_kernel<<<nblk, 256, 0, st>>>(dS, m, q.st, q.excl, q.idx, q.val);
    KL(c);
    return ABO_OK;
}
struct TopItem { uint64_t key; int64_t idx; double val; };
constexpr int64_t SEL_MIN_M = 65536;
static int device_topk_read(const SelSlot& q, int64_t K, int64_t idx_offset, std::vector<TopItem>& items, cudaStream_t st) {
    std::vector<long long> hi((size_t)K);
    std::vector<double> hv((size_t)K);
    CU(cudaMemcpyAsync(hi.data(), q.idx, sizeof(long long) * K, cudaMemcpyDeviceToHost, st));
    CU(cudaMemcpyAsync(hv.data(), q.val, sizeof(double) * K, cudaMemcpyDeviceToHost, st));
    CU(cudaStreamSynchronize(st));
    for (int64_t i = 0; i < K; ++i) items.push_back(TopItem{ordkey(hv[(size_t)i]), (int64_t)hi[(size_t)i] + idx_offset, hv[(size_t)i]});
    return ABO_OK;
}
static void topk_emit(std::vector<TopItem>& items, int64_t k, int64_t* top_idx, double* top_val) {
    std::sort(items.begin(), items.end(), [](const TopItem& a, const TopItem& b) { return a.key != b.key ? a.key > b.key : a.idx < b.idx; });
    const int64_t cnt = std::min<int64_t>(k, (int64_t)items.size());
    for (int64_t i = 0; i < cnt; ++i) { top_idx[i] = items[(size_t)i].idx; top_val[i] = items[(size_t)i].val; }
}

static int scores_select_readback(abo_ctx* c, const double* dS, int64_t m, double* h_scores, int64_t k, int64_t* top_idx, double* top_val);
static int acq_eval_common(abo_gp* g, int acq_id, const double* params, const double* dXc, int64_t m, double* d_scores,
                           double* h_scores, int64_t k, int64_t* top_idx, double* top_val) {
    abo_ctx* c = g->ctx;
    int rc;
    double* dS = d_scores;
    if (!dS && (rc = ws_get(c, WS_OUT_A, sizeof(double) * (size_t)m, (void**)&dS))) return rc;
    if ((rc = sweep_device(g, dXc, m, 0, acq_id, params, nullptr, nullptr, dS))) return rc;
    return scores_select_readback(c, dS, m, h_scores, k, top_idx, top_val);
}
static int scores_select_readback(abo_ctx* c, const double* dS, int64_t m, double* h_scores, int64_t k, int64_t* top_idx, double* top_val) {
    cudaStream_t st = c->stream;
    int rc;
    const int64_t K = std::min(k, m);
    if (K > 0 && m <= SEL_MIN_M) {
        double* hs = h_scores;
        if (!hs) { if ((rc = pinned_get(c, sizeof(double) * (size_t)m, (void**)&hs))) return rc; }
        CU(cudaMemcpyAsync(hs, dS, sizeof(double) * m, cudaMemcpyDeviceToHost, st));
        CU(cudaStreamSynchronize(st));
        auto better = [](const TopItem& a, const TopItem& b) { return a.key != b.key ? a.key > b.key : a.idx < b.idx; };
        std::vector<TopItem> keep;
        keep.reserve((size_t)K);
        int64_t i = 0;
        for (; i < K; ++i) keep.push_back(TopItem{ordkey(hs[i]), i, hs[i]});
        std::make_heap(keep.begin(), keep.end(), better);
        for (; i < m; ++i) {
            const uint64_t key = ordkey(hs[i]);
            if (key > keep.front().key) {
                std::pop_heap(keep.begin(), keep.end(), better);
                keep.back() = TopItem{key, i, hs[i]};
                std::push_heap(keep.begin(), keep.end(), better);
            }
        }
        std::sort(keep.begin(), keep.end(), better);
        for (int64_t q = 0; q < K; ++q) { top_idx[q] = keep[(size_t)q].idx; top_val[q] = keep[(size_t)q].val; }
        return ABO_OK;
    }
    SelSlot q{};
    if (K > 0) {
        if ((rc = sel_slot(c, 0, m, K, &q))) return rc;
        if ((rc = device_topk_launch(c, q, dS, m, K, st))) return rc;
    }
    if (h_scores) CU(cudaMemcpyAsync(h_scores, dS, sizeof(double) * m, cudaMemcpyDeviceToHost, st));
    if (K > 0) {
        std::vector<TopItem> items;
        items.reserve((size_t)K);
        if ((rc = device_topk_read(q, K, 0, items, st))) return rc;
        topk_emit(items, K, top_idx, top_val);
    } else {
        CU(cudaStreamSynchronize(st));
    }
    return ABO_OK;
}

static int acq_check(abo_gp* g, int acq_id, const double* params, const void* Xc, int64_t m, int64_t k,
                     int64_t* top_idx, double* top_val) {
    if (!g || !Xc || !params) return abo_fail(ABO_ERR_INVALID, "null argument");
    if (!g->fitted) return abo_fail(ABO_ERR_NOT_FITTED, "surrogate has no posterior (call update first)");
    if (acq_id < 0 || acq_id > 2) return abo_fail(ABO_ERR_INVALID, "unknown acquisition id %d", acq_id);
    if (m < 0 || k < 0) return abo_fail(ABO_ERR_INVALID, "negative size");
    if (k > 0 && (!top_idx || !top_val)) return abo_fail(ABO_ERR_INVALID, "top-k buffers are NULL");
    return ABO_OK;
}

static int sweep_host_pieces_run(abo_gp* g, const double* Xc, int64_t m, int acq_id, const double* params, double* h_mean,
                                 double* h_var, double* h_scores, int64_t k, int64_t* top_idx, double* top_val);
static int sweep_host_pieces(abo_gp* g, const double* Xc, int64_t m, int acq_id, const double* params, double* h_mean,
                             double* h_var, double* h_scores, int64_t k, int64_t* top_idx, double* top_val) {
    const int rc = sweep_host_pieces_run(g, Xc, m, acq_id, params, h_mean, h_var, h_scores, k, top_idx, top_val);
    if (rc) {
        const std::string keep = g_err;
        ctx_sync_all(g->ctx);
        cudaGetLastError();
        g_err = keep;
    }
    return rc;
}
static int sweep_host_pieces_run(abo_gp* g, const double* Xc, int64_t m, int acq_id, const double* params, double* h_mean,
                                 double* h_var, double* h_scores, int64_t k, int64_t* top_idx, double* top_val) {
    abo_ctx* c = g->ctx;
    cudaStream_t st = c->stream, sc = c->stream3;
    const int d = g->d;
    const int64_t piece = HOST_PIECE;
    const int64_t np = (m + piece - 1) / piece;
    int rc;
    double *dXc, *dA, *dB = nullptr;
    if ((rc = ws_get(c, WS_CAND, sizeof(double) * (size_t)m * d, (void**)&dXc))) return rc;
    if ((rc = ws_get(c, WS_OUT_A, sizeof(double) * (size_t)m, (void**)&dA))) return rc;
    if (acq_id < 0 && (rc = ws_get(c, WS_OUT_B, sizeof(double) * (size_t)m, (void**)&dB))) return rc;
    const int64_t Kp = (acq_id >= 0 && k > 0) ? std::min(k, piece) : 0;
    SelSlot slot[2] = {};
    if (Kp > 0) { if ((rc = sel_slot(c, 0, piece, Kp, &slot[0])) || (rc = sel_slot(c, 1, piece, Kp, &slot[1]))) return rc; }
    std::vector<TopItem> items;
    if (Kp > 0) items.reserve((size_t)(Kp * np));
    auto off = [&](int64_t i) { return i * piece; };
    auto cnt = [&](int64_t i) { return std::min(piece, m - i * piece); };
    auto drain = [&](int64_t i) -> int {
        double* hosts[2] = {acq_id >= 0 ? h_scores : h_mean, acq_id >= 0 ? nullptr : h_var};
        double* devs[2] = {dA, dB};
        if (!hosts[0] && !hosts[1] && Kp == 0) return ABO_OK;
        CU(cudaStreamWaitEvent(sc, c->ev_pc[i & 1], 0));
        for (int q = 0; q < 2; ++q)
            if (hosts[q]) CU(cudaMemcpyAsync(hosts[q] + off(i), devs[q] + off(i), sizeof(double) * cnt(i), cudaMemcpyDeviceToHost, sc));
        if (Kp > 0) return device_topk_read(slot[i & 1], std::min(Kp, cnt(i)), off(i), items, sc);
        CU(cudaStreamSynchronize(sc));
        return ABO_OK;
    };
    CU(cudaMemcpyAsync(dXc, Xc, sizeof(double) * cnt(0) * d, cudaMemcpyHostToDevice, sc));
    CU(cudaEventRecord(c->ev_h2d[0], sc));
    for (int64_t i = 0; i < np; ++i) {
        CU(cudaStreamWaitEvent(st, c->ev_h2d[i & 1], 0));
        if (acq_id >= 0) rc = sweep_device(g, dXc + off(i) * d, cnt(i), 0, acq_id, params, nullptr, nullptr, dA + off(i));
        else rc = sweep_device(g, dXc + off(i) * d, cnt(i), 0, -1, nullptr, dA + off(i), dB + off(i), nullptr);
        if (rc) return rc;
        if (Kp > 0 && (rc = device_topk_launch(c, slot[i & 1], dA + off(i), cnt(i), std::min(Kp, cnt(i)), st))) return rc;
        CU(cudaEventRecord(c->ev_pc[i & 1], st));
        if (i + 1 < np) {
            CU(cudaMemcpyAsync(dXc + off(i + 1) * d, Xc + off(i + 1) * d, sizeof(double) * cnt(i + 1) * d, cudaMemcpyHostToDevice, sc));
            CU(cudaEventRecord(c->ev_h2d[(i + 1) & 1], sc));
        }
        if (i >= 1 && (rc = drain(i - 1))) return rc;
    }
    if ((rc = drain(np - 1))) return rc;
    CU(cudaStreamSynchronize(st));
    if (Kp > 0) topk_emit(items, std::min(k, m), top_idx, top_val);
    return ABO_OK;
}

extern "C" int32_t abo_acq_eval(abo_gp* g, int32_t acq_id, const double* params, const double* Xc, int64_t m,
                                double* scores, int64_t k, int64_t* top_idx, double* top_val) {
    int rc = acq_check(g, acq_id, params, Xc, m, k, top_idx, top_val);
    if (rc) return rc;
    if (m == 0) return ABO_OK;
    abo_ctx* c = g->ctx;
    CU(cudaSetDevice(c->device));
    if (m > HOST_PIECE && !c->profile) return sweep_host_pieces(g, Xc, m, acq_id, params, nullptr, nullptr, scores, k, top_idx, top_val);
    double* dXc;
    if ((rc = ws_get(c, WS_CAND, sizeof(double) * (size_t)m * g->d, (void**)&dXc))) return rc;
    CU(cudaMemcpyAsync(dXc, Xc, sizeof(double) * m * g->d, cudaMemcpyHostToDevice, c->stream));
    return acq_eval_common(g, acq_id, params, dXc, m, nullptr, scores, k, top_idx, top_val);
}

extern "C" int32_t abo_acq_eval_dev(abo_gp* g, int32_t acq_id, const double* params, const double* d_Xc, int64_t m,
                                    double* d_scores, int64_t k, int64_t* top_idx, double* top_val) {
    int rc = acq_check(g, acq_id, params, d_Xc, m, k, top_idx, top_val);
    if (rc) return rc;
    if (m == 0) return ABO_OK;
    CU(cudaSetDevice(g->ctx->device));
    return acq_eval_common(g, acq_id, params, d_Xc, m, d_scores, nullptr, k, top_idx, top_val);
}

extern "C" int32_t abo_fill_distance(abo_ctx* c, const double* X, int64_t n, int32_t d, const double* S, int64_t m,
                                     double* h_fill) {
    if (!c || !X || !S || !h_fill) return abo_fail(ABO_ERR_INVALID, "null argument");
    if (n < 1 || m < 1 || d < 1 || d > 96) return abo_fail(ABO_ERR_INVALID, "bad sizes (d <= 96)");
    CU(cudaSetDevice(c->device));
    cudaStream_t st = c->stream;
    const int nblk = (int)((m + 255) / 256);
    double *dX, *dS, *dB;
    int rc;
    if ((rc = ws_get(c, WS_STAGE_X, sizeof(double) * (size_t)n * d, (void**)&dX))) return rc;
    if ((rc = ws_get(c, WS_CAND, sizeof(double) * (size_t)m * d, (void**)&dS))) return rc;
    if ((rc = ws_get(c, WS_OUT_A, sizeof(double) * (size_t)nblk, (void**)&dB))) return rc;
    CU(cudaMemcpyAsync(dX, X, sizeof(double) * n * d, cudaMemcpyHostToDevice, st));
    CU(cudaMemcpyAsync(dS, S, sizeof(double) * m * d, cudaMemcpyHostToDevice, st));
    fill_distance_kernel<<<nblk, 256, sizeof(double) * 256 * d, st>>>(dX, n, d, dS, m, dB);
    KL(c);
    std::vector<double> hb(nblk);
    CU(cudaMemcpyAsync(hb.data(), dB, sizeof(double) * nblk, cudaMemcpyDeviceToHost, st));
    CU(cudaStreamSynchronize(st));
    double r = 0.0;
    for (double v : hb) r = std::max(r, v);
    *h_fill = r;
    return ABO_OK;
}

extern "C" int32_t abo_potrf_dev(abo_ctx* c, double* d_A, int64_t n, int64_t ld, int64_t* info) {
    if (!c || !d_A) return abo_fail(ABO_ERR_INVALID, "null argument");
    if (n < 1 || n % NB != 0 || ld < n || ld % 2 != 0)
        return abo_fail(ABO_ERR_INVALID, "abo_potrf_dev needs n a multiple of 128 and an even ld >= n");
    CU(cudaSetDevice(c->device));
    const int T = (int)(n / NB);
    double* Dinv; int* dinfo;
    int rc;
    if ((rc = ws_get(c, WS_DINV, sizeof(double) * (size_t)T * NB * NB, (void**)&Dinv))) return rc;
    if ((rc = ws_get(c, WS_INFO, sizeof(int) * 16, (void**)&dinfo))) return rc;
    CU(cudaMemsetAsync(dinfo, 0, sizeof(int) * 16, c->stream));
    if ((rc = potrf_lookahead(c, d_A, n, ld, Dinv, dinfo))) return rc;
    int hinfo = 0;
    CU(cudaMemcpyAsync(&hinfo, dinfo, sizeof(int), cudaMemcpyDeviceToHost, c->stream));
    CU(cudaStreamSynchronize(c->stream));
    if (info) *info = hinfo;
    if (hinfo) return abo_fail(ABO_ERR_NOT_POSDEF, "matrix is not positive definite; Cholesky factorization failed at pivot %d", hinfo);
    return ABO_OK;
}

#include "abo_extra.cuh"
#include "abo_multi.cuh"
```

abstractbayesopt.jl_b200/csrc/abo_internal.h:

```cpp
#pragma once
#include <cstdint>
#include <cstring>
#include <utility>
#include <unordered_set>
#include <vector>
#include <cuda_runtime.h>

int abo_fail(int code, const char* fmt, ...);

#define CU(...)                                                                                       \
    do {                                                                                              \
        cudaError_t e_ = (__VA_ARGS__);                                                                      \
        if (e_ != cudaSuccess) {                                                                      \
            cudaGetLastError();                                                                       \
            return abo_fail(4 , "%s failed: %s (%s:%d)", #__VA_ARGS__, cudaGetErrorString(e_), \
                            __FILE__, __LINE__);                                                      \
        }                                                                                             \
    } while (0)

#define KL(ctx)                                                                                       \
    do {                                                                                              \
        (ctx)->launches++;                                                                            \
        cudaError_t e_ = cudaGetLastError();                                                          \
        if (e_ != cudaSuccess)                                                                        \
            return abo_fail(4, "kernel launch failed: %s (%s:%d)", cudaGetErrorString(e_), __FILE__, __LINE__); \
    } while (0)

enum WsSlot {
    WS_STAGE_X = 0, WS_STAGE_Y, WS_DINV, WS_INFO, WS_TRTRI, WS_VEC_PART, WS_KS, WS_PMEAN, WS_SUMSQ, WS_CAND,
    WS_OUT_A, WS_OUT_B, WS_NLML_K, WS_NLML_LINV, WS_NLML_W, WS_NLML_X, WS_NLML_VEC, WS_NLML_PAR, WS_APPEND,
    WS_TOPK, WS_SELECT, WS_GRAD_W, WS_GRAD_Z, WS_GRAD_PART, WS_GRAD_OUT, WS_TRTRI_U, WS_NLML_U,
    WS_SAMPLE_G, WS_SAMPLE_SIGMA, WS_SAMPLE_Z, WS_SAMPLE_F,
    WS_COUNT
};

struct WsBuf { void* ptr = nullptr; size_t bytes = 0; };

struct abo_ctx {
    int device = 0;
    int sms = 0;
    cudaStream_t stream = nullptr, stream2 = nullptr, stream3 = nullptr, stream4 = nullptr;
    cudaEvent_t ev_inv = nullptr;
    cudaEvent_t ev_p[3] = {nullptr, nullptr, nullptr};
    cudaEvent_t ev_a = nullptr, ev_b = nullptr;
    cudaEvent_t ev_h2d[2] = {nullptr, nullptr}, ev_pc[2] = {nullptr, nullptr};
    WsBuf ws[WS_COUNT];
    void* pinned = nullptr;
    size_t pinned_bytes = 0;
    int64_t launches = 0;
    bool profile = false;
    std::vector<cudaEvent_t> prof_events;
    size_t prof_used = 0;
    double prof_ms[3] = {0, 0, 0};
    int64_t prof_n[3] = {0, 0, 0};
    void* nccl_comm = nullptr;
    int rank = 0, nranks = 1;
    std::unordered_set<abo_gp*> live;
    struct GpBufSet { int64_t cap_pad, ldx; int d, p; double* ptr[7]; };
    std::vector<GpBufSet> gp_pool;
};

struct abo_gp {
    abo_ctx* ctx = nullptr;
    int kind = 0, d = 1, p = 1;
    double s = 1.0, scale = 1.0, noise = 0.0;
    std::vector<double> sv;
    bool ard = false;
    std::vector<double> mean_c;
    int64_t n = 0, N = 0, Npad = 0;
    int64_t cap_pad = 0, ld = 0, ldx = 0;
    bool fitted = false;
    double *dXsT = nullptr, *dL = nullptr, *dLinv = nullptr, *dAlpha = nullptr, *dBeta = nullptr,
           *dDelta = nullptr, *dMeanC = nullptr;
    int* share = nullptr;
};

static inline uint64_t ordkey(double v) {
    if (v != v) return ~0ull;
    uint64_t u;
    memcpy(&u, &v, 8);
    return (u >> 63) ? ~u : (u | 0x8000000000000000ull);
}

int gp_alloc(abo_gp* g, int64_t Npad, int64_t ldx);
int gp_unshare(abo_gp* g);
void gp_pool_clear(abo_ctx* c);
static inline bool gp_shared(const abo_gp* g) { return g->share && *g->share > 1; }
void ctx_sync_all(abo_ctx* c);
void ws_release(abo_ctx* c, int slot);
int ws_get(abo_ctx* c, int slot, size_t bytes, void** out);
int pinned_get(abo_ctx* c, size_t bytes, void** out);
int potrf_lookahead(abo_ctx* c, double* A, int64_t Npad, int64_t ld, double* Dinv, int* info, int notify_tile = 0, cudaStream_t notify_stream = nullptr);
int potrf_blocked(abo_ctx* c, double* A, int64_t Npad, int64_t ld, double* Dinv, int* info, int batch);
int trtri_tma(abo_ctx* c, const double* L, double* Linv, double* U, double* Wt, int64_t Npad, int64_t ld, int64_t strideM,
              const double* Dinv, int64_t strideD, int batch);
int solve_alpha(abo_ctx* c, const double* Linv, int64_t ld, int64_t N, const double* delta, double* beta,
                double* alpha, int64_t strideM, int64_t strideV, int batch);
void abo_nccl_teardown(abo_ctx* c);
int prof_mark(abo_ctx* c);
int prof_collect(abo_ctx* c);
```

abstractbayesopt.jl_b200/csrc/sweep_fused.cuh:

```cuda
#pragma once
#include <cstdint>
#include <cuda.h>
#include <cuda_runtime.h>
#include <type_traits>

#include "kernels.cuh"
#include "tma_pipe.cuh"

namespace abo {

constexpr int FS_STAGES = 5;
constexpr int FS_THREADS = 256 + 32;
constexpr int64_t FS_MAX_NPAD = 16384;

struct FusedParams {
    KSpec spec;
    AcqSpec acq;
    const double* XsT;
    int64_t ldx;
    int64_t n;
    int T;
    int Kld;
    const double* Xc;
    int64_t m;
    const double* beta;
    double* scratch;
    double* mean_out;
    double* var_out;
    double* score_out;
    int ntiles;
};

template <int DT>
constexpr int fused_smem_bytes() {
    return FS_STAGES * SW_STAGE_BYTES + 128 * DT * 8 + 2 * 4 * 128 * 8 + 2 * 128 * 8 + (2 * FS_STAGES + 2) * 8 + 128;
}

__device__ __forceinline__ void fence_proxy_async_global() { asm volatile("fence.proxy.async.global;\n" ::: "memory"); }
__device__ __forceinline__ void bar_consumers() { asm volatile("bar.sync 1, 256;\n" ::: "memory"); }

__device__ __forceinline__ void fused_stage_range(const double* __restrict__ a_s, const double* __restrict__ b_s, double (&acc)[4][8][2],
                                                  int ilo, int ihi) {
    switch (ilo * 5 + ihi) {
        case 0 * 5 + 4: dmma_stage<0, 4, 128>(a_s, b_s, acc); break;
        case 0 * 5 + 3: dmma_stage<0, 3, 128>(a_s, b_s, acc); break;
        case 0 * 5 + 2: dmma_stage<0, 2, 128>(a_s, b_s, acc); break;
        case 0 * 5 + 1: dmma_stage<0, 1, 128>(a_s, b_s, acc); break;
        case 1 * 5 + 4: dmma_stage<1, 4, 128>(a_s, b_s, acc); break;
        case 1 * 5 + 3: dmma_stage<1, 3, 128>(a_s, b_s, acc); break;
        case 1 * 5 + 2: dmma_stage<1, 2, 128>(a_s, b_s, acc); break;
        case 2 * 5 + 4: dmma_stage<2, 4, 128>(a_s, b_s, acc); break;
        case 2 * 5 + 3: dmma_stage<2, 3, 128>(a_s, b_s, acc); break;
        case 3 * 5 + 4: dmma_stage<3, 4, 128>(a_s, b_s, acc); break;
        default: break;
    }
}

template <int FAM>
__device__ __forceinline__ double phi_value(int kind, double u) {
    if (FAM == 0) return exp(-u / 2);
    const double r = sqrt(u);
    if (FAM == 1) {
        const double q5 = 2.23606797749978969641;
        const double v = (1 + q5 * r + u * (5.0 / 3.0)) * exp(-q5 * r);
        return (kind == K_AM52 && u < 1e-10) ? 1.0 - (5.0 / 6.0) * u : v;
    }
    const double q7 = 2.64575131106459059050;
    const double v = (1 + q7 * r + u * (14.0 / 5.0) + (7.0 / 15.0) * q7 * r * u) * exp(-q7 * r);
    return (kind == K_AM72 && u < 1e-10) ? 1.0 - (7.0 / 10.0) * u : v;
}

template <int DT>
__global__ void __launch_bounds__(FS_THREADS, 1)
sweep_fused_kernel(const __grid_constant__ CUtensorMap tmA, const __grid_constant__ CUtensorMap tmB, const FusedParams p) {
    extern __shared__ __align__(128) unsigned char fs_smem[];
    double* stage_base = reinterpret_cast<double*>(fs_smem);
    double* sc = reinterpret_cast<double*>(fs_smem + FS_STAGES * SW_STAGE_BYTES);
    double* red = sc + 128 * DT;
    double* qacc = red + 2 * 4 * 128;
    double* macc = qacc + 128;
    uint64_t* full = reinterpret_cast<uint64_t*>(macc + 128);
    uint64_t* empty = full + FS_STAGES;
    uint64_t* built = empty + FS_STAGES;

    const int tid = threadIdx.x, lane = tid & 31, warp = tid >> 5;
    const int G = gridDim.x, b = blockIdx.x;
    const int ntl = (b < p.ntiles) ? (p.ntiles - b + G - 1) / G : 0;
    const int nk_max = p.Kld / 16;

    if (tid == 0) {
        for (int s = 0; s < FS_STAGES; ++s) { mbar_init(&full[s], 1); mbar_init(&empty[s], 8); }
        mbar_init(&built[0], 1); mbar_init(&built[1], 1);
        asm volatile("fence.mbarrier_init.release.cluster;\n" ::: "memory");
    }
    if (tid < 128) { qacc[tid] = 0.0; macc[tid] = 0.0; }
    __syncthreads();

    if (warp == 8) {
        if (lane == 0) {
            int stage = 0;
            uint32_t phase = 0;
            for (int j = 0; j < ntl; ++j) {
                mbar_wait(&built[j & 1], (uint32_t)((j >> 1) & 1));
                const int brow = (b * 2 + (j & 1)) * 128;
                for (int ib = 0; ib < p.T; ++ib) {
                    const int nk = min((ib + 1) * 8, nk_max);
                    const int m0 = ib * 128;
                    for (int kt = 0; kt < nk; ++kt) {
                        mbar_wait(&empty[stage], phase ^ 1);
                        tma_stage_load(stage_base + (size_t)stage * (2 * SW_OPER_DOUBLES), &full[stage], &tmA, kt * 16, m0,
                                       &tmB, kt * 16, brow);
                        if (++stage == FS_STAGES) { stage = 0; phase ^= 1; }
                    }
                }
            }
        }
        return;
    }

    const int q = warp & 3, wn = (warp >> 2) * 64;
    const int fr = lane >> 2, fk = lane & 3;
    const int d = p.spec.d;
    const int64_t n = p.n;
    double* my_scratch = p.scratch + (size_t)b * 2 * 128 * p.Kld;

    {
        const int padw = p.Kld - (int)n;
        for (int e = tid; e < 2 * 128 * padw; e += 256) my_scratch[(size_t)(e / padw) * p.Kld + n + (e % padw)] = 0.0;
    }

    constexpr int BCU = 8;
    auto build = [&](int j) {
        const int64_t c_base = ((int64_t)b + (int64_t)j * G) * 128;
        double* tile = my_scratch + (size_t)(j & 1) * 128 * p.Kld;
        for (int e = tid; e < 128 * DT; e += 256) {
            const int c = e / DT, k = e - c * DT;
            const int64_t gc = c_base + c;
            sc[e] = (k < d && gc < p.m) ? p.spec.sk(k) * p.Xc[gc * d + k] : 0.0;
        }
        bar_consumers();
        const int nitems = (int)((n + 31) / 32) * 4;
        auto items = [&](auto fam_tag) {
            constexpr int FAM = decltype(fam_tag)::value;
            constexpr bool PREF = DT <= 12;
            double xn[PREF ? DT : 1];
            if (PREF) {
                const int64_t i0 = (int64_t)(warp >> 2) * 32 + lane;
#pragma unroll
                for (int k = 0; k < DT; ++k) xn[PREF ? k : 0] = (k < d && i0 < n && warp < nitems) ? p.XsT[(int64_t)k * p.ldx + i0] : 0.0;
            }
            for (int item = warp; item < nitems; item += 8) {
                const int64_t i = (int64_t)(item >> 2) * 32 + lane;
                const int c0 = (item & 3) * 32;
                const bool live = i < n;
                double x[DT];
                if (PREF) {
#pragma unroll
                    for (int k = 0; k < DT; ++k) x[k] = xn[PREF ? k : 0];
                    const int64_t i2 = (int64_t)((item + 8) >> 2) * 32 + lane;
                    const bool nxt = (item + 8 < nitems) && i2 < n;
#pragma unroll
                    for (int k = 0; k < DT; ++k) xn[PREF ? k : 0] = (k < d && nxt) ? p.XsT[(int64_t)k * p.ldx + i2] : 0.0;
                } else {
#pragma unroll
                    for (int k = 0; k < DT; ++k) x[k] = (k < d && live) ? p.XsT[(int64_t)k * p.ldx + i] : 0.0;
                }
                double* col = tile + i;
#pragma unroll 1
                for (int c = c0; c < c0 + 32; c += BCU) {
                    double u[BCU];
#pragma unroll
                    for (int r = 0; r < BCU; ++r) u[r] = 0.0;
#pragma unroll
                    for (int k = 0; k < DT; ++k) {
#pragma unroll
                        for (int r = 0; r < BCU; ++r) { const double df = x[k] - sc[(c + r) * DT + k]; u[r] = fma(df, df, u[r]); }
                    }
#pragma unroll
                    for (int r = 0; r < BCU; ++r) {
                        const double v = p.spec.scale * phi_value<FAM>(p.spec.kind, u[r]);
                        if (live) col[(size_t)(c + r) * p.Kld] = v;
                    }
                }
            }
        };
        const int kind = p.spec.kind;
        if (kind == K_SE) items(std::integral_constant<int, 0>{});
        else if (kind == K_M52 || kind == K_AM52 || kind == K_ADM52) items(std::integral_constant<int, 1>{});
        else items(std::integral_constant<int, 2>{});
        fence_proxy_async_global();
        __threadfence();
        bar_consumers();
        if (tid == 0) mbar_arrive(&built[j & 1]);
    };

    int stage = 0;
    uint32_t phase = 0;
    for (int j = -1; j < ntl; ++j) {
        if (j + 1 < ntl) build(j + 1);
        if (j < 0) continue;
        const int64_t c_base = ((int64_t)b + (int64_t)j * G) * 128;
        for (int ib = 0; ib < p.T; ++ib) {
            const int nk = min((ib + 1) * 8, nk_max);
            const int m0 = ib * 128;
            const int rows = (int)min((int64_t)128, n - m0);
            const int nfrag = (rows + 7) >> 3;
            const int ni = max(0, min(4, (nfrag - q + 3) >> 2));
            double acc[4][8][2];
#pragma unroll
            for (int i = 0; i < 4; ++i)
#pragma unroll
                for (int jj = 0; jj < 8; ++jj) { acc[i][jj][0] = 0.0; acc[i][jj][1] = 0.0; }
            const int a_off = ((8 * q + fr) << 2) + fk;
            const int b_off = SW_OPER_DOUBLES + ((wn + fr) << 2) + fk;
            const int nk_full = (rows == 128) ? min(nk, ib * 8) : 0;
            for (int kt = 0; kt < nk_full; ++kt) {
                mbar_wait(&full[stage], phase);
                const double* st = stage_base + (size_t)stage * (2 * SW_OPER_DOUBLES);
                dmma_stage<0, 4, 128>(st + a_off, st + b_off, acc);
                __syncwarp();
                if (lane == 0) mbar_arrive(&empty[stage]);
                if (++stage == FS_STAGES) { stage = 0; phase ^= 1; }
            }
            for (int kt = nk_full; kt < nk; ++kt) {
                mbar_wait(&full[stage], phase);
                const double* st = stage_base + (size_t)stage * (2 * SW_OPER_DOUBLES);
                const int t = kt - ib * 8;
                const int ilo = t > 0 ? max(0, (2 * t - q + 3) >> 2) : 0;
                fused_stage_range(st + a_off, st + b_off, acc, ilo, ni);
                __syncwarp();
                if (lane == 0) mbar_arrive(&empty[stage]);
                if (++stage == FS_STAGES) { stage = 0; phase ^= 1; }
            }
            double bt[4];
#pragma unroll
            for (int i = 0; i < 4; ++i) bt[i] = p.beta[m0 + 8 * (4 * i + q) + fr];
#pragma unroll
            for (int jj = 0; jj < 8; ++jj) {
#pragma unroll
                for (int e = 0; e < 2; ++e) {
                    double s2 = 0.0, sm = 0.0;
#pragma unroll
                    for (int i = 0; i < 4; ++i) { s2 = fma(acc[i][jj][e], acc[i][jj][e], s2); sm = fma(acc[i][jj][e], bt[i], sm); }
                    s2 += __shfl_xor_sync(0xffffffffu, s2, 4);  sm += __shfl_xor_sync(0xffffffffu, sm, 4);
                    s2 += __shfl_xor_sync(0xffffffffu, s2, 8);  sm += __shfl_xor_sync(0xffffffffu, sm, 8);
                    s2 += __shfl_xor_sync(0xffffffffu, s2, 16); sm += __shfl_xor_sync(0xffffffffu, sm, 16);
                    if (fr == 0) {
                        const int col = wn + jj * 8 + 2 * fk + e;
                        red[q * 128 + col] = s2;
                        red[512 + q * 128 + col] = sm;
                    }
                }
            }
            bar_consumers();
            if (tid < 128) {
                qacc[tid] += ((red[tid] + red[128 + tid]) + red[256 + tid]) + red[384 + tid];
                macc[tid] += ((red[512 + tid] + red[640 + tid]) + red[768 + tid]) + red[896 + tid];
            }
            bar_consumers();
        }
        if (tid < 128) {
            const int64_t gc = c_base + tid;
            if (gc < p.m) {
                const double mu = macc[tid] + p.acq.mean_c;
                const double var = (p.acq.kss - qacc[tid]) + JITTER;
                if (p.mean_out) p.mean_out[gc] = mu;
                if (p.var_out) p.var_out[gc] = var;
                if (p.score_out && p.acq.acq >= 0) p.score_out[gc] = acq_value(p.acq, mu, var);
            }
            qacc[tid] = 0.0; macc[tid] = 0.0;
        }
    }
}

}
```

Before: 529,000.

## Emulate FP64 posterior sweep via Ozaki int8 slices on tcgen05 UMMA

Replaces the DMMA-based fused sweep for large training sets with an Ozaki-scheme kernel. The kernel splits the L-inverse rows and the cross-kernel columns into 8 int8 digit slices and accumulates the slice products with tcgen05 int8 MMA into tensor memory. A new pre-pass kernel converts L-inverse into per-row-scaled digit planes, and TMA loads 3D digit tiles. The aim is to move the dominant triangular GEMM from slow FP64 tensor-core throughput to much faster int8 UMMA. In exchange it adds digit-conversion work and extra memory per call, plus possible accuracy differences. The old DMMA path is kept for small Npad.

```diff
diff --git a/abstractbayesopt.jl_b200/csrc/abo_api.cu b/abstractbayesopt.jl_b200/csrc/abo_api.cu
--- a/abstractbayesopt.jl_b200/csrc/abo_api.cu
+++ b/abstractbayesopt.jl_b200/csrc/abo_api.cu
@@ -15,6 +15,7 @@
 #include "gemm_dmma.cuh"
 #include "kernels.cuh"
 #include "sweep_fused.cuh"
+#include "sweep_fused_dmma.cuh"
 #include "gemm_tma.cuh"
 #include "sample.cuh"
 #include "abo_internal.h"
@@ -47,7 +48,8 @@
     CU(cudaFuncSetAttribute(syrk_tma_kernel, cudaFuncAttributeMaxDynamicSharedMemorySize, SY_SMEM_BYTES));
     CU(cudaFuncSetAttribute(gemm_tma_kernel<EPI_STORE>, cudaFuncAttributeMaxDynamicSharedMemorySize, tg_smem_bytes<EPI_STORE>()));
     CU(cudaFuncSetAttribute(gemm_tma_kernel<EPI_COLSUMSQ>, cudaFuncAttributeMaxDynamicSharedMemorySize, tg_smem_bytes<EPI_COLSUMSQ>()));
-#define ABO_FS_CFG(DT) CU(cudaFuncSetAttribute(sweep_fused_kernel<DT>, cudaFuncAttributeMaxDynamicSharedMemorySize, fused_smem_bytes<DT>()))
+#define ABO_FS_CFG(DT) CU(cudaFuncSetAttribute(sweep_fused_kernel<DT>, cudaFuncAttributeMaxDynamicSharedMemorySize, fused_smem_bytes<DT>())); \
+    CU(cudaFuncSetAttribute(sweep_fused_dmma_kernel<DT>, cudaFuncAttributeMaxDynamicSharedMemorySize, fused_dmma_smem_bytes<DT>()))
     ABO_FS_CFG(4); ABO_FS_CFG(8); ABO_FS_CFG(12); ABO_FS_CFG(16); ABO_FS_CFG(20); ABO_FS_CFG(24); ABO_FS_CFG(32);
 #undef ABO_FS_CFG
     return ABO_OK;
@@ -893,11 +895,11 @@
 static bool fused_applies(const abo_gp* g, int bo) {
     return g->p == 1 && bo == 0 && g->d <= 32 && g->Npad <= FS_MAX_NPAD;
 }
-static int sweep_fused_device(abo_gp* g, const double* dXc, int64_t m, const AcqSpec& a, double* d_mean, double* d_var,
+static int sweep_fused_dmma_device(abo_gp* g, const double* dXc, int64_t m, const AcqSpec& a, double* d_mean, double* d_var,
                               double* d_score) {
     abo_ctx* c = g->ctx;
     cudaStream_t st = c->stream;
-    FusedParams fp;
+    FusedDmmaParams fp;
     fp.spec = gp_spec(g); fp.acq = a;
     fp.XsT = g->dXsT; fp.ldx = g->ldx; fp.n = g->n;
     fp.T = (int)((g->n + NB - 1) / NB);
@@ -913,6 +915,65 @@
     if ((rc = make_tmap_k4(&tmB, fp.scratch, fp.Kld, (int64_t)c->sms * 2 * NB, fp.Kld))) return rc;
     if ((rc = prof_mark(c)) || (rc = prof_mark(c))) return rc;
     if ((rc = prof_mark(c))) return rc;
+#define ABO_FS_RUN(DT) sweep_fused_dmma_kernel<DT><<<grid, FSD_THREADS, fused_dmma_smem_bytes<DT>(), st>>>(tmA, tmB, fp)
+    const int d = g->d;
+    if (d <= 4) ABO_FS_RUN(4); else if (d <= 8) ABO_FS_RUN(8); else if (d <= 12) ABO_FS_RUN(12); else if (d <= 16) ABO_FS_RUN(16);
+    else if (d <= 20) ABO_FS_RUN(20); else if (d <= 24) ABO_FS_RUN(24); else ABO_FS_RUN(32);
+#undef ABO_FS_RUN
+    KL(c);
+    if ((rc = prof_mark(c))) return rc;
+    if ((rc = prof_mark(c)) || (rc = prof_mark(c))) return rc;
+    if (c->profile && c->prof_used >= 6 * 512) {
+        CU(cudaStreamSynchronize(st));
+        if ((rc = prof_collect(c))) return rc;
+    }
+    return ABO_OK;
+}
+
+static int make_tmap_digits(CUtensorMap* map, const int8_t* base, int64_t K, int64_t rows, int box_rows) {
+    EncodeTiledFn fn = get_encode_fn();
+    if (!fn) return abo_fail(ABO_ERR_CUDA, "cuTensorMapEncodeTiled is not available from this driver");
+    cuuint64_t dims[3] = {(cuuint64_t)K, (cuuint64_t)rows, (cuuint64_t)OZ_S};
+    cuuint64_t strides[2] = {(cuuint64_t)K, (cuuint64_t)(K * rows)};
+    cuuint32_t box[3] = {32, (cuuint32_t)box_rows, (cuuint32_t)OZ_S};
+    cuuint32_t estr[3] = {1, 1, 1};
+    CUresult r = fn(map, CU_TENSOR_MAP_DATA_TYPE_UINT8, 3, (void*)base, dims, strides, box, estr, CU_TENSOR_MAP_INTERLEAVE_NONE,
+                    CU_TENSOR_MAP_SWIZZLE_32B, CU_TENSOR_MAP_L2_PROMOTION_L2_256B, CU_TENSOR_MAP_FLOAT_OOB_FILL_NONE);
+    if (r != CUDA_SUCCESS) return abo_fail(ABO_ERR_CUDA, "cuTensorMapEncodeTiled failed with CUresult %d", (int)r);
+    return ABO_OK;
+}
+static int sweep_fused_int8_device(abo_gp* g, const double* dXc, int64_t m, const AcqSpec& a, double* d_mean, double* d_var,
+                              double* d_score) {
+    abo_ctx* c = g->ctx;
+    cudaStream_t st = c->stream;
+    const int64_t Npad = g->Npad;
+    FusedParams fp;
+    fp.spec = gp_spec(g); fp.acq = a;
+    fp.XsT = g->dXsT; fp.ldx = g->ldx; fp.n = g->n;
+    fp.T = (int)((g->n + OZ_ROWS - 1) / OZ_ROWS);
+    fp.Kld = (int)((g->n + 31) / 32 * 32);
+    fp.Xc = dXc; fp.m = m; fp.alpha = g->dAlpha;
+    int e_k = 0;
+    std::frexp(fp.spec.scale, &e_k);
+    fp.kup = std::ldexp(1.0, 62 - e_k);
+    fp.wscale = std::ldexp(1.0, e_k - 62 + 56);
+    fp.mean_out = d_mean; fp.var_out = d_var; fp.score_out = d_score;
+    fp.ntiles = (int)((m + OZ_NC - 1) / OZ_NC);
+    fp.srows = (int64_t)c->sms * 2 * OZ_NC;
+    const int grid = std::min(c->sms, fp.ntiles);
+    int rc;
+    if ((rc = ws_get(c, WS_KS, (size_t)OZ_S * fp.srows * fp.Kld, (void**)&fp.scratch))) return rc;
+    int8_t* ldig;
+    if ((rc = ws_get(c, WS_LINV_DIGITS, (size_t)OZ_S * Npad * Npad + sizeof(double) * Npad, (void**)&ldig))) return rc;
+    double* rscale = reinterpret_cast<double*>(ldig + (size_t)OZ_S * Npad * Npad);
+    fp.rscale = rscale;
+    CUtensorMap tmA, tmB;
+    if ((rc = make_tmap_digits(&tmA, ldig, Npad, Npad, OZ_ROWS))) return rc;
+    if ((rc = make_tmap_digits(&tmB, fp.scratch, fp.Kld, fp.srows, OZ_NC))) return rc;
+    if ((rc = prof_mark(c))) return rc;
+    linv_digits_kernel<<<(unsigned)(fp.T * OZ_ROWS / 8), 256, 0, st>>>(g->dLinv, g->ld, g->n, fp.Kld, Npad, ldig, rscale);
+    KL(c);
+    if ((rc = prof_mark(c)) || (rc = prof_mark(c))) return rc;
 #define ABO_FS_RUN(DT) sweep_fused_kernel<DT><<<grid, FS_THREADS, fused_smem_bytes<DT>(), st>>>(tmA, tmB, fp)
     const int d = g->d;
     if (d <= 4) ABO_FS_RUN(4); else if (d <= 8) ABO_FS_RUN(8); else if (d <= 12) ABO_FS_RUN(12); else if (d <= 16) ABO_FS_RUN(16);
@@ -939,7 +1000,9 @@
         a0.p1 = (params && acq != ACQ_UCB && acq >= 0) ? params[1] : 0.0;
         a0.mean_c = g->mean_c[bo];
         a0.kss = g->scale;
-        if (fused_applies(g, bo)) return sweep_fused_device(g, dXc, m, a0, d_mean, d_var, d_score);
+        if (fused_applies(g, bo))
+            return g->Npad >= FS_INT8_MIN_NPAD ? sweep_fused_int8_device(g, dXc, m, a0, d_mean, d_var, d_score)
+                                               : sweep_fused_dmma_device(g, dXc, m, a0, d_mean, d_var, d_score);
     }
     const int64_t Npad = g->Npad;
     const int T = (int)(Npad / NB);
diff --git a/abstractbayesopt.jl_b200/csrc/abo_internal.h b/abstractbayesopt.jl_b200/csrc/abo_internal.h
--- a/abstractbayesopt.jl_b200/csrc/abo_internal.h
+++ b/abstractbayesopt.jl_b200/csrc/abo_internal.h
@@ -31,6 +31,7 @@
     WS_OUT_A, WS_OUT_B, WS_NLML_K, WS_NLML_LINV, WS_NLML_W, WS_NLML_X, WS_NLML_VEC, WS_NLML_PAR, WS_APPEND,
     WS_TOPK, WS_SELECT, WS_GRAD_W, WS_GRAD_Z, WS_GRAD_PART, WS_GRAD_OUT, WS_TRTRI_U, WS_NLML_U,
     WS_SAMPLE_G, WS_SAMPLE_SIGMA, WS_SAMPLE_Z, WS_SAMPLE_F,
+    WS_LINV_DIGITS,
     WS_COUNT
 };
 
diff --git a/abstractbayesopt.jl_b200/csrc/sweep_fused.cuh b/abstractbayesopt.jl_b200/csrc/sweep_fused.cuh
--- a/abstractbayesopt.jl_b200/csrc/sweep_fused.cuh
+++ b/abstractbayesopt.jl_b200/csrc/sweep_fused.cuh
@@ -5,13 +5,20 @@
 #include <type_traits>
 
 #include "kernels.cuh"
-#include "tma_pipe.cuh"
+#include "umma.cuh"
 
 namespace abo {
 
-constexpr int FS_STAGES = 5;
-constexpr int FS_THREADS = 256 + 32;
+constexpr int OZ_S = 8;
+constexpr int OZ_NC = 64;
+constexpr int OZ_ROWS = 128;
+constexpr int FS_STAGES = 4;
+constexpr int FS_A_BYTES = OZ_S * OZ_ROWS * 32;
+constexpr int FS_B_BYTES = OZ_S * OZ_NC * 32;
+constexpr int FS_STAGE_BYTES = FS_A_BYTES + FS_B_BYTES;
+constexpr int FS_THREADS = 256;
 constexpr int64_t FS_MAX_NPAD = 16384;
+constexpr int64_t FS_INT8_MIN_NPAD = 1024;
 
 struct FusedParams {
     KSpec spec;
@@ -23,8 +30,12 @@
     int Kld;
     const double* Xc;
     int64_t m;
-    const double* beta;
-    double* scratch;
+    const double* alpha;
+    const double* rscale;
+    double kup;
+    double wscale;
+    int8_t* scratch;
+    int64_t srows;
     double* mean_out;
     double* var_out;
     double* score_out;
@@ -33,26 +44,53 @@
 
 template <int DT>
 constexpr int fused_smem_bytes() {
-    return FS_STAGES * SW_STAGE_BYTES + 128 * DT * 8 + 2 * 4 * 128 * 8 + 2 * 128 * 8 + (2 * FS_STAGES + 2) * 8 + 128;
+    return 1024 + FS_STAGES * FS_STAGE_BYTES + (OZ_NC * DT + OZ_NC + 2 * OZ_NC + 4 * OZ_NC + OZ_NC) * 8 + (2 * FS_STAGES + 6) * 8 + 16;
 }
 
 __device__ __forceinline__ void fence_proxy_async_global() { asm volatile("fence.proxy.async.global;\n" ::: "memory"); }
-__device__ __forceinline__ void bar_consumers() { asm volatile("bar.sync 1, 256;\n" ::: "memory"); }
-
-__device__ __forceinline__ void fused_stage_range(const double* __restrict__ a_s, const double* __restrict__ b_s, double (&acc)[4][8][2],
-                                                  int ilo, int ihi) {
-    switch (ilo * 5 + ihi) {
-        case 0 * 5 + 4: dmma_stage<0, 4, 128>(a_s, b_s, acc); break;
-        case 0 * 5 + 3: dmma_stage<0, 3, 128>(a_s, b_s, acc); break;
-        case 0 * 5 + 2: dmma_stage<0, 2, 128>(a_s, b_s, acc); break;
-        case 0 * 5 + 1: dmma_stage<0, 1, 128>(a_s, b_s, acc); break;
-        case 1 * 5 + 4: dmma_stage<1, 4, 128>(a_s, b_s, acc); break;
-        case 1 * 5 + 3: dmma_stage<1, 3, 128>(a_s, b_s, acc); break;
-        case 1 * 5 + 2: dmma_stage<1, 2, 128>(a_s, b_s, acc); break;
-        case 2 * 5 + 4: dmma_stage<2, 4, 128>(a_s, b_s, acc); break;
-        case 2 * 5 + 3: dmma_stage<2, 3, 128>(a_s, b_s, acc); break;
-        case 3 * 5 + 4: dmma_stage<3, 4, 128>(a_s, b_s, acc); break;
-        default: break;
+__device__ __forceinline__ void bar_drain() { asm volatile("bar.sync 1, 128;\n" ::: "memory"); }
+__device__ __forceinline__ void bar_build() { asm volatile("bar.sync 2, 64;\n" ::: "memory"); }
+
+__device__ __forceinline__ void oz_split(double x, int8_t (&dg)[OZ_S]) {
+    long long M = __double2ll_rn(x);
+#pragma unroll
+    for (int t = OZ_S - 1; t > 0; --t) {
+        const long long lo = ((M + 128) & 255) - 128;
+        dg[t] = (int8_t)lo;
+        M = (M - lo) >> 8;
+    }
+    dg[0] = (int8_t)M;
+}
+
+__global__ void __launch_bounds__(256) linv_digits_kernel(const double* __restrict__ L, int64_t ld, int64_t n, int Kld, int64_t Npad,
+                                                          int8_t* __restrict__ dig, double* __restrict__ rscale) {
+    const int64_t i = (int64_t)blockIdx.x * 8 + (threadIdx.x >> 5);
+    const int lane = threadIdx.x & 31;
+    const int64_t kend = min((i / OZ_ROWS + 1) * OZ_ROWS, (int64_t)Kld);
+    const int64_t klive = i < n ? i + 1 : 0;
+    const double* row = L + i * ld;
+    double mx = 0.0;
+    for (int64_t k = lane; k < klive; k += 32) mx = fmax(mx, fabs(row[k]));
+#pragma unroll
+    for (int o = 16; o > 0; o >>= 1) mx = fmax(mx, __shfl_xor_sync(0xffffffffu, mx, o));
+    int e = 0;
+    if (mx > 0.0) frexp(mx, &e);
+    const double up = ldexp(1.0, 62 - e);
+    if (lane == 0) rscale[i] = ldexp(1.0, e - 62);
+    for (int64_t k0 = 4 * lane; k0 < kend; k0 += 128) {
+        uint32_t w[OZ_S];
+#pragma unroll
+        for (int t = 0; t < OZ_S; ++t) w[t] = 0;
+#pragma unroll
+        for (int r = 0; r < 4; ++r) {
+            const double v = (k0 + r < klive) ? row[k0 + r] : 0.0;
+            int8_t dg[OZ_S];
+            oz_split(v * up, dg);
+#pragma unroll
+            for (int t = 0; t < OZ_S; ++t) w[t] |= (uint32_t)(uint8_t)dg[t] << (8 * r);
+        }
+#pragma unroll
+        for (int t = 0; t < OZ_S; ++t) *reinterpret_cast<uint32_t*>(dig + ((int64_t)t * Npad + i) * Npad + k0) = w[t];
     }
 }
 
@@ -73,43 +111,55 @@
 template <int DT>
 __global__ void __launch_bounds__(FS_THREADS, 1)
 sweep_fused_kernel(const __grid_constant__ CUtensorMap tmA, const __grid_constant__ CUtensorMap tmB, const FusedParams p) {
-    extern __shared__ __align__(128) unsigned char fs_smem[];
-    double* stage_base = reinterpret_cast<double*>(fs_smem);
-    double* sc = reinterpret_cast<double*>(fs_smem + FS_STAGES * SW_STAGE_BYTES);
-    double* red = sc + 128 * DT;
-    double* qacc = red + 2 * 4 * 128;
-    double* macc = qacc + 128;
-    uint64_t* full = reinterpret_cast<uint64_t*>(macc + 128);
+    extern __shared__ unsigned char fs_raw[];
+    unsigned char* stages = fs_raw + ((1024 - (smem_u32(fs_raw) & 1023)) & 1023);
+    double* sc = reinterpret_cast<double*>(stages + FS_STAGES * FS_STAGE_BYTES);
+    double* mpart = sc + OZ_NC * DT;
+    double* macc = mpart + OZ_NC;
+    double* red = macc + 2 * OZ_NC;
+    double* qacc = red + 4 * OZ_NC;
+    uint64_t* full = reinterpret_cast<uint64_t*>(qacc + OZ_NC);
     uint64_t* empty = full + FS_STAGES;
-    uint64_t* built = empty + FS_STAGES;
+    uint64_t* tfull = empty + FS_STAGES;
+    uint64_t* tempty = tfull + 1;
+    uint64_t* built = tempty + 1;
+    uint64_t* freed = built + 2;
+    uint32_t* tslot = reinterpret_cast<uint32_t*>(freed + 2);
 
     const int tid = threadIdx.x, lane = tid & 31, warp = tid >> 5;
     const int G = gridDim.x, b = blockIdx.x;
     const int ntl = (b < p.ntiles) ? (p.ntiles - b + G - 1) / G : 0;
-    const int nk_max = p.Kld / 16;
+    const int nkb_max = p.Kld / 32;
 
     if (tid == 0) {
-        for (int s = 0; s < FS_STAGES; ++s) { mbar_init(&full[s], 1); mbar_init(&empty[s], 8); }
-        mbar_init(&built[0], 1); mbar_init(&built[1], 1);
+        for (int s = 0; s < FS_STAGES; ++s) { mbar_init(&full[s], 1); mbar_init(&empty[s], 1); }
+        mbar_init(tfull, 1); mbar_init(tempty, 4);
+        for (int s = 0; s < 2; ++s) { mbar_init(&built[s], 1); mbar_init(&freed[s], 1); }
         asm volatile("fence.mbarrier_init.release.cluster;\n" ::: "memory");
     }
-    if (tid < 128) { qacc[tid] = 0.0; macc[tid] = 0.0; }
+    if (warp == 0) tmem_alloc<OZ_S * OZ_NC>(tslot);
+    if (tid < OZ_NC) qacc[tid] = 0.0;
+    if (tid < OZ_NC) mpart[tid] = 0.0;
+    tmem_fence_before();
     __syncthreads();
-
-    if (warp == 8) {
+    tmem_fence_after();
+    const uint32_t tbase = *tslot;
+
+    if (warp == 6) {
         if (lane == 0) {
             int stage = 0;
             uint32_t phase = 0;
             for (int j = 0; j < ntl; ++j) {
                 mbar_wait(&built[j & 1], (uint32_t)((j >> 1) & 1));
-                const int brow = (b * 2 + (j & 1)) * 128;
+                const int brow = (b * 2 + (j & 1)) * OZ_NC;
                 for (int ib = 0; ib < p.T; ++ib) {
-                    const int nk = min((ib + 1) * 8, nk_max);
-                    const int m0 = ib * 128;
-                    for (int kt = 0; kt < nk; ++kt) {
+                    const int nkb = min((ib + 1) * (OZ_ROWS / 32), nkb_max);
+                    for (int kb = 0; kb < nkb; ++kb) {
                         mbar_wait(&empty[stage], phase ^ 1);
-                        tma_stage_load(stage_base + (size_t)stage * (2 * SW_OPER_DOUBLES), &full[stage], &tmA, kt * 16, m0,
-                                       &tmB, kt * 16, brow);
+                        unsigned char* st = stages + (size_t)stage * FS_STAGE_BYTES;
+                        mbar_expect_tx(&full[stage], FS_STAGE_BYTES);
+                        tma_load_3d(st, &tmA, kb * 32, ib * OZ_ROWS, 0, &full[stage]);
+                        tma_load_3d(st + FS_A_BYTES, &tmB, kb * 32, brow, 0, &full[stage]);
                         if (++stage == FS_STAGES) { stage = 0; phase ^= 1; }
                     }
                 }
@@ -118,54 +168,64 @@
         return;
     }
 
-    const int q = warp & 3, wn = (warp >> 2) * 64;
-    const int fr = lane >> 2, fk = lane & 3;
+    if (warp == 7) {
+        if (lane == 0) {
+            constexpr uint32_t idesc = umma_idesc_i8<OZ_ROWS, OZ_NC>();
+            int stage = 0, rt = 0;
+            uint32_t phase = 0;
+            for (int j = 0; j < ntl; ++j) {
+                for (int ib = 0; ib < p.T; ++ib, ++rt) {
+                    const int nkb = min((ib + 1) * (OZ_ROWS / 32), nkb_max);
+                    mbar_wait(tempty, (uint32_t)((rt & 1) ^ 1));
+                    tmem_fence_after();
+                    for (int kb = 0; kb < nkb; ++kb) {
+                        mbar_wait(&full[stage], phase);
+                        tmem_fence_after();
+                        const unsigned char* st = stages + (size_t)stage * FS_STAGE_BYTES;
+#pragma unroll
+                        for (int a = 0; a < OZ_S; ++a) {
+                            const uint64_t ad = umma_desc_sw32(st + a * (OZ_ROWS * 32));
+#pragma unroll
+                            for (int q = 0; q < OZ_S - a; ++q)
+                                umma_i8(tbase + (uint32_t)((a + q) * OZ_NC), ad, umma_desc_sw32(st + FS_A_BYTES + q * (OZ_NC * 32)), idesc,
+                                        kb > 0 || a > 0);
+                        }
+                        umma_commit(&empty[stage]);
+                        if (++stage == FS_STAGES) { stage = 0; phase ^= 1; }
+                    }
+                    umma_commit(tfull);
+                }
+            }
+        }
+        return;
+    }
+
     const int d = p.spec.d;
     const int64_t n = p.n;
-    double* my_scratch = p.scratch + (size_t)b * 2 * 128 * p.Kld;
-
-    {
-        const int padw = p.Kld - (int)n;
-        for (int e = tid; e < 2 * 128 * padw; e += 256) my_scratch[(size_t)(e / padw) * p.Kld + n + (e % padw)] = 0.0;
-    }
-
-    constexpr int BCU = 8;
-    auto build = [&](int j) {
-        const int64_t c_base = ((int64_t)b + (int64_t)j * G) * 128;
-        double* tile = my_scratch + (size_t)(j & 1) * 128 * p.Kld;
-        for (int e = tid; e < 128 * DT; e += 256) {
-            const int c = e / DT, k = e - c * DT;
-            const int64_t gc = c_base + c;
-            sc[e] = (k < d && gc < p.m) ? p.spec.sk(k) * p.Xc[gc * d + k] : 0.0;
-        }
-        bar_consumers();
-        const int nitems = (int)((n + 31) / 32) * 4;
-        auto items = [&](auto fam_tag) {
+    if (warp >= 4) {
+        const int bt = tid - 128, bw = warp - 4;
+        const size_t plane = (size_t)p.srows * p.Kld;
+        int8_t* my_scratch = p.scratch + (size_t)b * 2 * OZ_NC * p.Kld;
+        {
+            const int padw = p.Kld - (int)n;
+            for (int e = bt; e < OZ_S * 2 * OZ_NC * padw; e += 64) {
+                const int r = e / padw, t = r / (2 * OZ_NC);
+                my_scratch[t * plane + (size_t)(r - t * 2 * OZ_NC) * p.Kld + n + (e - r * padw)] = 0;
+            }
+        }
+        constexpr int BCU = 4;
+        const int nitems = (int)((n + 31) / 32) * 2;
+        auto items = [&](auto fam_tag, int8_t* tile) {
             constexpr int FAM = decltype(fam_tag)::value;
-            constexpr bool PREF = DT <= 12;
-            double xn[PREF ? DT : 1];
-            if (PREF) {
-                const int64_t i0 = (int64_t)(warp >> 2) * 32 + lane;
-#pragma unroll
-                for (int k = 0; k < DT; ++k) xn[PREF ? k : 0] = (k < d && i0 < n && warp < nitems) ? p.XsT[(int64_t)k * p.ldx + i0] : 0.0;
-            }
-            for (int item = warp; item < nitems; item += 8) {
-                const int64_t i = (int64_t)(item >> 2) * 32 + lane;
-                const int c0 = (item & 3) * 32;
+            for (int item = bw; item < nitems; item += 2) {
+                const int64_t i = (int64_t)(item >> 1) * 32 + lane;
+                const int c0 = (item & 1) * 32;
                 const bool live = i < n;
+                const double al = live ? p.alpha[i] : 0.0;
                 double x[DT];
-                if (PREF) {
-#pragma unroll
-                    for (int k = 0; k < DT; ++k) x[k] = xn[PREF ? k : 0];
-                    const int64_t i2 = (int64_t)((item + 8) >> 2) * 32 + lane;
-                    const bool nxt = (item + 8 < nitems) && i2 < n;
-#pragma unroll
-                    for (int k = 0; k < DT; ++k) xn[PREF ? k : 0] = (k < d && nxt) ? p.XsT[(int64_t)k * p.ldx + i2] : 0.0;
-                } else {
-#pragma unroll
-                    for (int k = 0; k < DT; ++k) x[k] = (k < d && live) ? p.XsT[(int64_t)k * p.ldx + i] : 0.0;
-                }
-                double* col = tile + i;
+#pragma unroll
+                for (int k = 0; k < DT; ++k) x[k] = (k < d && live) ? p.XsT[(int64_t)k * p.ldx + i] : 0.0;
+                int8_t* col = tile + i;
 #pragma unroll 1
                 for (int c = c0; c < c0 + 32; c += BCU) {
                     double u[BCU];
@@ -179,98 +239,107 @@
 #pragma unroll
                     for (int r = 0; r < BCU; ++r) {
                         const double v = p.spec.scale * phi_value<FAM>(p.spec.kind, u[r]);
-                        if (live) col[(size_t)(c + r) * p.Kld] = v;
+                        double pm = live ? v * al : 0.0;
+                        if (live) {
+                            int8_t dg[OZ_S];
+                            oz_split(v * p.kup, dg);
+                            int8_t* dst = col + (size_t)(c + r) * p.Kld;
+#pragma unroll
+                            for (int t = 0; t < OZ_S; ++t, dst += plane) *dst = dg[t];
+                        }
+#pragma unroll
+                        for (int o = 16; o > 0; o >>= 1) pm += __shfl_xor_sync(0xffffffffu, pm, o);
+                        if (lane == 0) mpart[c + r] += pm;
                     }
                 }
             }
         };
-        const int kind = p.spec.kind;
-        if (kind == K_SE) items(std::integral_constant<int, 0>{});
-        else if (kind == K_M52 || kind == K_AM52 || kind == K_ADM52) items(std::integral_constant<int, 1>{});
-        else items(std::integral_constant<int, 2>{});
-        fence_proxy_async_global();
-        __threadfence();
-        bar_consumers();
-        if (tid == 0) mbar_arrive(&built[j & 1]);
-    };
-
-    int stage = 0;
-    uint32_t phase = 0;
-    for (int j = -1; j < ntl; ++j) {
-        if (j + 1 < ntl) build(j + 1);
-        if (j < 0) continue;
-        const int64_t c_base = ((int64_t)b + (int64_t)j * G) * 128;
-        for (int ib = 0; ib < p.T; ++ib) {
-            const int nk = min((ib + 1) * 8, nk_max);
-            const int m0 = ib * 128;
-            const int rows = (int)min((int64_t)128, n - m0);
-            const int nfrag = (rows + 7) >> 3;
-            const int ni = max(0, min(4, (nfrag - q + 3) >> 2));
-            double acc[4][8][2];
-#pragma unroll
-            for (int i = 0; i < 4; ++i)
-#pragma unroll
-                for (int jj = 0; jj < 8; ++jj) { acc[i][jj][0] = 0.0; acc[i][jj][1] = 0.0; }
-            const int a_off = ((8 * q + fr) << 2) + fk;
-            const int b_off = SW_OPER_DOUBLES + ((wn + fr) << 2) + fk;
-            const int nk_full = (rows == 128) ? min(nk, ib * 8) : 0;
-            for (int kt = 0; kt < nk_full; ++kt) {
-                mbar_wait(&full[stage], phase);
-                const double* st = stage_base + (size_t)stage * (2 * SW_OPER_DOUBLES);
-                dmma_stage<0, 4, 128>(st + a_off, st + b_off, acc);
-                __syncwarp();
-                if (lane == 0) mbar_arrive(&empty[stage]);
-                if (++stage == FS_STAGES) { stage = 0; phase ^= 1; }
-            }
-            for (int kt = nk_full; kt < nk; ++kt) {
-                mbar_wait(&full[stage], phase);
-                const double* st = stage_base + (size_t)stage * (2 * SW_OPER_DOUBLES);
-                const int t = kt - ib * 8;
-                const int ilo = t > 0 ? max(0, (2 * t - q + 3) >> 2) : 0;
-                fused_stage_range(st + a_off, st + b_off, acc, ilo, ni);
-                __syncwarp();
-                if (lane == 0) mbar_arrive(&empty[stage]);
-                if (++stage == FS_STAGES) { stage = 0; phase ^= 1; }
-            }
-            double bt[4];
-#pragma unroll
-            for (int i = 0; i < 4; ++i) bt[i] = p.beta[m0 + 8 * (4 * i + q) + fr];
-#pragma unroll
-            for (int jj = 0; jj < 8; ++jj) {
-#pragma unroll
-                for (int e = 0; e < 2; ++e) {
-                    double s2 = 0.0, sm = 0.0;
-#pragma unroll
-                    for (int i = 0; i < 4; ++i) { s2 = fma(acc[i][jj][e], acc[i][jj][e], s2); sm = fma(acc[i][jj][e], bt[i], sm); }
-                    s2 += __shfl_xor_sync(0xffffffffu, s2, 4);  sm += __shfl_xor_sync(0xffffffffu, sm, 4);
-                    s2 += __shfl_xor_sync(0xffffffffu, s2, 8);  sm += __shfl_xor_sync(0xffffffffu, sm, 8);
-                    s2 += __shfl_xor_sync(0xffffffffu, s2, 16); sm += __shfl_xor_sync(0xffffffffu, sm, 16);
-                    if (fr == 0) {
-                        const int col = wn + jj * 8 + 2 * fk + e;
-                        red[q * 128 + col] = s2;
-                        red[512 + q * 128 + col] = sm;
-                    }
-                }
-            }
-            bar_consumers();
-            if (tid < 128) {
-                qacc[tid] += ((red[tid] + red[128 + tid]) + red[256 + tid]) + red[384 + tid];
-                macc[tid] += ((red[512 + tid] + red[640 + tid]) + red[768 + tid]) + red[896 + tid];
-            }
-            bar_consumers();
-        }
-        if (tid < 128) {
+        for (int j = 0; j < ntl; ++j) {
+            const int slot = j & 1;
+            if (j >= 2) mbar_wait(&freed[slot], (uint32_t)(((j - 2) >> 1) & 1));
+            const int64_t c_base = ((int64_t)b + (int64_t)j * G) * OZ_NC;
+            for (int e = bt; e < OZ_NC * DT; e += 64) {
+                const int c = e / DT, k = e - c * DT;
+                const int64_t gc = c_base + c;
+                sc[e] = (k < d && gc < p.m) ? p.spec.sk(k) * p.Xc[gc * d + k] : 0.0;
+            }
+            bar_build();
+            int8_t* tile = my_scratch + (size_t)slot * OZ_NC * p.Kld;
+            const int kind = p.spec.kind;
+            if (kind == K_SE) items(std::integral_constant<int, 0>{}, tile);
+            else if (kind == K_M52 || kind == K_AM52 || kind == K_ADM52) items(std::integral_constant<int, 1>{}, tile);
+            else items(std::integral_constant<int, 2>{}, tile);
+            fence_proxy_async_global();
+            __threadfence();
+            bar_build();
+            macc[slot * OZ_NC + bt] = mpart[bt];
+            mpart[bt] = 0.0;
+            bar_build();
+            if (bt == 0) mbar_arrive(&built[slot]);
+        }
+        return;
+    }
+
+    const uint32_t tlane = tbase + ((uint32_t)(32 * warp) << 16);
+    int rt = 0;
+    for (int j = 0; j < ntl; ++j) {
+        const int slot = j & 1;
+        const int64_t c_base = ((int64_t)b + (int64_t)j * G) * OZ_NC;
+        for (int ib = 0; ib < p.T; ++ib, ++rt) {
+            mbar_wait(tfull, (uint32_t)(rt & 1));
+            tmem_fence_after();
+            const double s_i = p.rscale[ib * OZ_ROWS + tid] * p.wscale;
+#pragma unroll 1
+            for (int ch = 0; ch < OZ_NC / 16; ++ch) {
+                double x[16];
+#pragma unroll
+                for (int l = 0; l < OZ_S; ++l) {
+                    int32_t D[16];
+                    tmem_ld16(tlane + (uint32_t)(l * OZ_NC + ch * 16), D);
+                    tmem_wait_ld();
+#pragma unroll
+                    for (int c = 0; c < 16; ++c) x[c] = l ? fma(x[c], 256.0, (double)D[c]) : (double)D[c];
+                }
+#pragma unroll
+                for (int c = 0; c < 16; ++c) { const double w = x[c] * s_i; x[c] = w * w; }
+#pragma unroll
+                for (int h = 16, nv = 8; h >= 2; h >>= 1, nv >>= 1) {
+                    const bool up = (lane & h) != 0;
+#pragma unroll
+                    for (int v = 0; v < nv; ++v) {
+                        const double send = up ? x[v] : x[v + nv];
+                        const double keep = up ? x[v + nv] : x[v];
+                        x[v] = keep + __shfl_xor_sync(0xffffffffu, send, h);
+                    }
+                }
+                const double s = x[0] + __shfl_xor_sync(0xffffffffu, x[0], 1);
+                if ((lane & 1) == 0)
+                    red[warp * OZ_NC + ch * 16 + ((lane >> 4) & 1) * 8 + ((lane >> 3) & 1) * 4 + ((lane >> 2) & 1) * 2 + ((lane >> 1) & 1)] = s;
+            }
+            tmem_fence_before();
+            __syncwarp();
+            if (lane == 0) mbar_arrive(tempty);
+            bar_drain();
+            if (tid < OZ_NC) qacc[tid] += ((red[tid] + red[OZ_NC + tid]) + red[2 * OZ_NC + tid]) + red[3 * OZ_NC + tid];
+            bar_drain();
+        }
+        mbar_wait(&built[slot], (uint32_t)((j >> 1) & 1));
+        if (tid < OZ_NC) {
             const int64_t gc = c_base + tid;
             if (gc < p.m) {
-                const double mu = macc[tid] + p.acq.mean_c;
-                const double var = (p.acq.kss - qacc[tid]) + JITTER;
+                const double mu = macc[slot * OZ_NC + tid] + p.acq.mean_c;
+                double var = (p.acq.kss - qacc[tid]) + JITTER;
+                if (mu != mu) var = mu;
                 if (p.mean_out) p.mean_out[gc] = mu;
                 if (p.var_out) p.var_out[gc] = var;
                 if (p.score_out && p.acq.acq >= 0) p.score_out[gc] = acq_value(p.acq, mu, var);
             }
-            qacc[tid] = 0.0; macc[tid] = 0.0;
-        }
-    }
-}
-
-}
+            qacc[tid] = 0.0;
+        }
+        bar_drain();
+        if (tid == 0) mbar_arrive(&freed[slot]);
+    }
+    if (warp == 0) tmem_dealloc<OZ_S * OZ_NC>(tbase);
+}
+
+}
diff --git a/abstractbayesopt.jl_b200/csrc/sweep_fused_dmma.cuh b/abstractbayesopt.jl_b200/csrc/sweep_fused_dmma.cuh
--- /dev/null
+++ b/abstractbayesopt.jl_b200/csrc/sweep_fused_dmma.cuh
@@ -0,0 +1,261 @@
+#pragma once
+#include <cstdint>
+#include <cuda.h>
+#include <cuda_runtime.h>
+#include <type_traits>
+
+#include "kernels.cuh"
+#include "sweep_fused.cuh"
+#include "tma_pipe.cuh"
+
+namespace abo {
+
+constexpr int FSD_STAGES = 5;
+constexpr int FSD_THREADS = 256 + 32;
+
+struct FusedDmmaParams {
+    KSpec spec;
+    AcqSpec acq;
+    const double* XsT;
+    int64_t ldx;
+    int64_t n;
+    int T;
+    int Kld;
+    const double* Xc;
+    int64_t m;
+    const double* beta;
+    double* scratch;
+    double* mean_out;
+    double* var_out;
+    double* score_out;
+    int ntiles;
+};
+
+template <int DT>
+constexpr int fused_dmma_smem_bytes() {
+    return FSD_STAGES * SW_STAGE_BYTES + 128 * DT * 8 + 2 * 4 * 128 * 8 + 2 * 128 * 8 + (2 * FSD_STAGES + 2) * 8 + 128;
+}
+
+__device__ __forceinline__ void bar_consumers() { asm volatile("bar.sync 1, 256;\n" ::: "memory"); }
+
+__device__ __forceinline__ void fused_stage_range(const double* __restrict__ a_s, const double* __restrict__ b_s, double (&acc)[4][8][2],
+                                                  int ilo, int ihi) {
+    switch (ilo * 5 + ihi) {
+        case 0 * 5 + 4: dmma_stage<0, 4, 128>(a_s, b_s, acc); break;
+        case 0 * 5 + 3: dmma_stage<0, 3, 128>(a_s, b_s, acc); break;
+        case 0 * 5 + 2: dmma_stage<0, 2, 128>(a_s, b_s, acc); break;
+        case 0 * 5 + 1: dmma_stage<0, 1, 128>(a_s, b_s, acc); break;
+        case 1 * 5 + 4: dmma_stage<1, 4, 128>(a_s, b_s, acc); break;
+        case 1 * 5 + 3: dmma_stage<1, 3, 128>(a_s, b_s, acc); break;
+        case 1 * 5 + 2: dmma_stage<1, 2, 128>(a_s, b_s, acc); break;
+        case 2 * 5 + 4: dmma_stage<2, 4, 128>(a_s, b_s, acc); break;
+        case 2 * 5 + 3: dmma_stage<2, 3, 128>(a_s, b_s, acc); break;
+        case 3 * 5 + 4: dmma_stage<3, 4, 128>(a_s, b_s, acc); break;
+        default: break;
+    }
+}
+
+template <int DT>
+__global__ void __launch_bounds__(FSD_THREADS, 1)
+sweep_fused_dmma_kernel(const __grid_constant__ CUtensorMap tmA, const __grid_constant__ CUtensorMap tmB, const FusedDmmaParams p) {
+    extern __shared__ __align__(128) unsigned char fs_smem[];
+    double* stage_base = reinterpret_cast<double*>(fs_smem);
+    double* sc = reinterpret_cast<double*>(fs_smem + FSD_STAGES * SW_STAGE_BYTES);
+    double* red = sc + 128 * DT;
+    double* qacc = red + 2 * 4 * 128;
+    double* macc = qacc + 128;
+    uint64_t* full = reinterpret_cast<uint64_t*>(macc + 128);
+    uint64_t* empty = full + FSD_STAGES;
+    uint64_t* built = empty + FSD_STAGES;
+
+    const int tid = threadIdx.x, lane = tid & 31, warp = tid >> 5;
+    const int G = gridDim.x, b = blockIdx.x;
+    const int ntl = (b < p.ntiles) ? (p.ntiles - b + G - 1) / G : 0;
+    const int nk_max = p.Kld / 16;
+
+    if (tid == 0) {
+        for (int s = 0; s < FSD_STAGES; ++s) { mbar_init(&full[s], 1); mbar_init(&empty[s], 8); }
+        mbar_init(&built[0], 1); mbar_init(&built[1], 1);
+        asm volatile("fence.mbarrier_init.release.cluster;\n" ::: "memory");
+    }
+    if (tid < 128) { qacc[tid] = 0.0; macc[tid] = 0.0; }
+    __syncthreads();
+
+    if (warp == 8) {
+        if (lane == 0) {
+            int stage = 0;
+            uint32_t phase = 0;
+            for (int j = 0; j < ntl; ++j) {
+                mbar_wait(&built[j & 1], (uint32_t)((j >> 1) & 1));
+                const int brow = (b * 2 + (j & 1)) * 128;
+                for (int ib = 0; ib < p.T; ++ib) {
+                    const int nk = min((ib + 1) * 8, nk_max);
+                    const int m0 = ib * 128;
+                    for (int kt = 0; kt < nk; ++kt) {
+                        mbar_wait(&empty[stage], phase ^ 1);
+                        tma_stage_load(stage_base + (size_t)stage * (2 * SW_OPER_DOUBLES), &full[stage], &tmA, kt * 16, m0,
+                                       &tmB, kt * 16, brow);
+                        if (++stage == FSD_STAGES) { stage = 0; phase ^= 1; }
+                    }
+                }
+            }
+        }
+        return;
+    }
+
+    const int q = warp & 3, wn = (warp >> 2) * 64;
+    const int fr = lane >> 2, fk = lane & 3;
+    const int d = p.spec.d;
+    const int64_t n = p.n;
+    double* my_scratch = p.scratch + (size_t)b * 2 * 128 * p.Kld;
+
+    {
+        const int padw = p.Kld - (int)n;
+        for (int e = tid; e < 2 * 128 * padw; e += 256) my_scratch[(size_t)(e / padw) * p.Kld + n + (e % padw)] = 0.0;
+    }
+
+    constexpr int BCU = 8;
+    auto build = [&](int j) {
+        const int64_t c_base = ((int64_t)b + (int64_t)j * G) * 128;
+        double* tile = my_scratch + (size_t)(j & 1) * 128 * p.Kld;
+        for (int e = tid; e < 128 * DT; e += 256) {
+            const int c = e / DT, k = e - c * DT;
+            const int64_t gc = c_base + c;
+            sc[e] = (k < d && gc < p.m) ? p.spec.sk(k) * p.Xc[gc * d + k] : 0.0;
+        }
+        bar_consumers();
+        const int nitems = (int)((n + 31) / 32) * 4;
+        auto items = [&](auto fam_tag) {
+            constexpr int FAM = decltype(fam_tag)::value;
+            constexpr bool PREF = DT <= 12;
+            double xn[PREF ? DT : 1];
+            if (PREF) {
+                const int64_t i0 = (int64_t)(warp >> 2) * 32 + lane;
+#pragma unroll
+                for (int k = 0; k < DT; ++k) xn[PREF ? k : 0] = (k < d && i0 < n && warp < nitems) ? p.XsT[(int64_t)k * p.ldx + i0] : 0.0;
+            }
+            for (int item = warp; item < nitems; item += 8) {
+                const int64_t i = (int64_t)(item >> 2) * 32 + lane;
+                const int c0 = (item & 3) * 32;
+                const bool live = i < n;
+                double x[DT];
+                if (PREF) {
+#pragma unroll
+                    for (int k = 0; k < DT; ++k) x[k] = xn[PREF ? k : 0];
+                    const int64_t i2 = (int64_t)((item + 8) >> 2) * 32 + lane;
+                    const bool nxt = (item + 8 < nitems) && i2 < n;
+#pragma unroll
+                    for (int k = 0; k < DT; ++k) xn[PREF ? k : 0] = (k < d && nxt) ? p.XsT[(int64_t)k * p.ldx + i2] : 0.0;
+                } else {
+#pragma unroll
+                    for (int k = 0; k < DT; ++k) x[k] = (k < d && live) ? p.XsT[(int64_t)k * p.ldx + i] : 0.0;
+                }
+                double* col = tile + i;
+#pragma unroll 1
+                for (int c = c0; c < c0 + 32; c += BCU) {
+                    double u[BCU];
+#pragma unroll
+                    for (int r = 0; r < BCU; ++r) u[r] = 0.0;
+#pragma unroll
+                    for (int k = 0; k < DT; ++k) {
+#pragma unroll
+                        for (int r = 0; r < BCU; ++r) { const double df = x[k] - sc[(c + r) * DT + k]; u[r] = fma(df, df, u[r]); }
+                    }
+#pragma unroll
+                    for (int r = 0; r < BCU; ++r) {
+                        const double v = p.spec.scale * phi_value<FAM>(p.spec.kind, u[r]);
+                        if (live) col[(size_t)(c + r) * p.Kld] = v;
+                    }
+                }
+            }
+        };
+        const int kind = p.spec.kind;
+        if (kind == K_SE) items(std::integral_constant<int, 0>{});
+        else if (kind == K_M52 || kind == K_AM52 || kind == K_ADM52) items(std::integral_constant<int, 1>{});
+        else items(std::integral_constant<int, 2>{});
+        fence_proxy_async_global();
+        __threadfence();
+        bar_consumers();
+        if (tid == 0) mbar_arrive(&built[j & 1]);
+    };
+
+    int stage = 0;
+    uint32_t phase = 0;
+    for (int j = -1; j < ntl; ++j) {
+        if (j + 1 < ntl) build(j + 1);
+        if (j < 0) continue;
+        const int64_t c_base = ((int64_t)b + (int64_t)j * G) * 128;
+        for (int ib = 0; ib < p.T; ++ib) {
+            const int nk = min((ib + 1) * 8, nk_max);
+            const int m0 = ib * 128;
+            const int rows = (int)min((int64_t)128, n - m0);
+            const int nfrag = (rows + 7) >> 3;
+            const int ni = max(0, min(4, (nfrag - q + 3) >> 2));
+            double acc[4][8][2];
+#pragma unroll
+            for (int i = 0; i < 4; ++i)
+#pragma unroll
+                for (int jj = 0; jj < 8; ++jj) { acc[i][jj][0] = 0.0; acc[i][jj][1] = 0.0; }
+            const int a_off = ((8 * q + fr) << 2) + fk;
+            const int b_off = SW_OPER_DOUBLES + ((wn + fr) << 2) + fk;
+            const int nk_full = (rows == 128) ? min(nk, ib * 8) : 0;
+            for (int kt = 0; kt < nk_full; ++kt) {
+                mbar_wait(&full[stage], phase);
+                const double* st = stage_base + (size_t)stage * (2 * SW_OPER_DOUBLES);
+                dmma_stage<0, 4, 128>(st + a_off, st + b_off, acc);
+                __syncwarp();
+                if (lane == 0) mbar_arrive(&empty[stage]);
+                if (++stage == FSD_STAGES) { stage = 0; phase ^= 1; }
+            }
+            for (int kt = nk_full; kt < nk; ++kt) {
+                mbar_wait(&full[stage], phase);
+                const double* st = stage_base + (size_t)stage * (2 * SW_OPER_DOUBLES);
+                const int t = kt - ib * 8;
+                const int ilo = t > 0 ? max(0, (2 * t - q + 3) >> 2) : 0;
+                fused_stage_range(st + a_off, st + b_off, acc, ilo, ni);
+                __syncwarp();
+                if (lane == 0) mbar_arrive(&empty[stage]);
+                if (++stage == FSD_STAGES) { stage = 0; phase ^= 1; }
+            }
+            double bt[4];
+#pragma unroll
+            for (int i = 0; i < 4; ++i) bt[i] = p.beta[m0 + 8 * (4 * i + q) + fr];
+#pragma unroll
+            for (int jj = 0; jj < 8; ++jj) {
+#pragma unroll
+                for (int e = 0; e < 2; ++e) {
+                    double s2 = 0.0, sm = 0.0;
+#pragma unroll
+                    for (int i = 0; i < 4; ++i) { s2 = fma(acc[i][jj][e], acc[i][jj][e], s2); sm = fma(acc[i][jj][e], bt[i], sm); }
+                    s2 += __shfl_xor_sync(0xffffffffu, s2, 4);  sm += __shfl_xor_sync(0xffffffffu, sm, 4);
+                    s2 += __shfl_xor_sync(0xffffffffu, s2, 8);  sm += __shfl_xor_sync(0xffffffffu, sm, 8);
+                    s2 += __shfl_xor_sync(0xffffffffu, s2, 16); sm += __shfl_xor_sync(0xffffffffu, sm, 16);
+                    if (fr == 0) {
+                        const int col = wn + jj * 8 + 2 * fk + e;
+                        red[q * 128 + col] = s2;
+                        red[512 + q * 128 + col] = sm;
+                    }
+                }
+            }
+            bar_consumers();
+            if (tid < 128) {
+                qacc[tid] += ((red[tid] + red[128 + tid]) + red[256 + tid]) + red[384 + tid];
+                macc[tid] += ((red[512 + tid] + red[640 + tid]) + red[768 + tid]) + red[896 + tid];
+            }
+            bar_consumers();
+        }
+        if (tid < 128) {
+            const int64_t gc = c_base + tid;
+            if (gc < p.m) {
+                const double mu = macc[tid] + p.acq.mean_c;
+                const double var = (p.acq.kss - qacc[tid]) + JITTER;
+                if (p.mean_out) p.mean_out[gc] = mu;
+                if (p.var_out) p.var_out[gc] = var;
+                if (p.score_out && p.acq.acq >= 0) p.score_out[gc] = acq_value(p.acq, mu, var);
+            }
+            qacc[tid] = 0.0; macc[tid] = 0.0;
+        }
+    }
+}
+
+}
diff --git a/abstractbayesopt.jl_b200/csrc/umma.cuh b/abstractbayesopt.jl_b200/csrc/umma.cuh
--- /dev/null
+++ b/abstractbayesopt.jl_b200/csrc/umma.cuh
@@ -0,0 +1,62 @@
+#pragma once
+#include <cstdint>
+
+#include "tma_pipe.cuh"
+
+namespace abo {
+
+__device__ __forceinline__ uint64_t umma_desc_sw32(const void* smem) {
+    const uint64_t addr = smem_u32(smem);
+    return ((addr >> 4) & 0x3FFFull) | (1ull << 16) | ((uint64_t)(256 >> 4) << 32) | (1ull << 46) | (6ull << 61);
+}
+
+template <int M, int N>
+__host__ __device__ constexpr uint32_t umma_idesc_i8() {
+    static_assert(M == 128 && N % 16 == 0 && N >= 16 && N <= 256, "cta_group::1 int8 MMA shape");
+    return (2u << 4) | (1u << 7) | (1u << 10) | ((uint32_t)(N >> 3) << 17) | ((uint32_t)(M >> 4) << 24);
+}
+
+__device__ __forceinline__ void umma_i8(uint32_t d_tmem, uint64_t a_desc, uint64_t b_desc, uint32_t idesc, bool accumulate) {
+    asm volatile(
+        "{\n"
+        ".reg .pred p;\n"
+        "setp.ne.b32 p, %4, 0;\n"
+        "tcgen05.mma.cta_group::1.kind::i8 [%0], %1, %2, %3, p;\n"
+        "}\n" ::"r"(d_tmem), "l"(a_desc), "l"(b_desc), "r"(idesc), "r"((uint32_t)accumulate)
+        : "memory");
+}
+
+__device__ __forceinline__ void umma_commit(uint64_t* bar) {
+    asm volatile("tcgen05.commit.cta_group::1.mbarrier::arrive::one.shared::cluster.b64 [%0];\n" ::"r"(smem_u32(bar)) : "memory");
+}
+
+__device__ __forceinline__ void tmem_fence_before() { asm volatile("tcgen05.fence::before_thread_sync;\n" ::: "memory"); }
+__device__ __forceinline__ void tmem_fence_after() { asm volatile("tcgen05.fence::after_thread_sync;\n" ::: "memory"); }
+
+template <int NCOLS>
+__device__ __forceinline__ void tmem_alloc(uint32_t* slot) {
+    asm volatile("tcgen05.alloc.cta_group::1.sync.aligned.shared::cta.b32 [%0], %1;\n" ::"r"(smem_u32(slot)), "n"(NCOLS) : "memory");
+    asm volatile("tcgen05.relinquish_alloc_permit.cta_group::1.sync.aligned;\n" ::: "memory");
+}
+template <int NCOLS>
+__device__ __forceinline__ void tmem_dealloc(uint32_t base) {
+    asm volatile("tcgen05.dealloc.cta_group::1.sync.aligned.b32 %0, %1;\n" ::"r"(base), "n"(NCOLS) : "memory");
+}
+
+__device__ __forceinline__ void tmem_ld16(uint32_t taddr, int32_t (&v)[16]) {
+    asm volatile(
+        "tcgen05.ld.sync.aligned.32x32b.x16.b32 {%0, %1, %2, %3, %4, %5, %6, %7, %8, %9, %10, %11, %12, %13, %14, %15}, [%16];\n"
+        : "=r"(v[0]), "=r"(v[1]), "=r"(v[2]), "=r"(v[3]), "=r"(v[4]), "=r"(v[5]), "=r"(v[6]), "=r"(v[7]), "=r"(v[8]),
+          "=r"(v[9]), "=r"(v[10]), "=r"(v[11]), "=r"(v[12]), "=r"(v[13]), "=r"(v[14]), "=r"(v[15])
+        : "r"(taddr));
+}
+__device__ __forceinline__ void tmem_wait_ld() { asm volatile("tcgen05.wait::ld.sync.aligned;\n" ::: "memory"); }
+
+__device__ __forceinline__ void tma_load_3d(void* dst, const CUtensorMap* map, int c0, int c1, int c2, uint64_t* bar) {
+    asm volatile(
+        "cp.async.bulk.tensor.3d.shared::cluster.global.mbarrier::complete_tx::bytes [%0], [%1, {%2, %3, %4}], [%5];\n" ::
+            "r"(smem_u32(dst)), "l"(map), "r"(c0), "r"(c1), "r"(c2), "r"(smem_u32(bar))
+        : "memory");
+}
+
+}
```

After: 743,800 (median of 6 runs). +40.6%, better.
